# mcychan/nQuant.android

Hardware: AMD Instinct MI355X
Metric: Mpixels/sec, 4096x4096 RGBA -> 256-colour PnnLAB + dither (higher is better)
Workload: dtype f64

## Files before the change

### include/nquant_abi.h

```cpp
#ifndef NQUANT_ABI_H
#define NQUANT_ABI_H
#include <stdint.h>

#ifdef __cplusplus
extern "C" {
#endif

#define NQ_ABI_VERSION 1

typedef struct nq_handle nq_handle;

enum nq_kind { NQ_KIND_RGB = 0,
               NQ_KIND_LAB = 1 };

enum nq_mode {
    NQ_MODE_REFERENCE_SEQUENTIAL = 0,
    NQ_MODE_PARALLEL_TILED = 1,
    NQ_MODE_LOOKUP_ONLY = 2
};

enum nq_status {
    NQ_OK = 0,
    NQ_ERR_INVALID = -1,
    NQ_ERR_HIP = -2,
    NQ_ERR_UNSUPPORTED = -3,
    NQ_ERR_REFERENCE_THROWS = -4,
    NQ_ERR_NO_DEVICE = -5,
    NQ_ERR_TIME_LIMIT = -6
};

typedef struct nq_params {
    int32_t kind;
    int32_t nMaxColors;
    int32_t hasSemiTransparency;
    int32_t transparentPixelIndex;
    int32_t transparentColor;
    int32_t isNano;
    int32_t texicab;
    int32_t quan_rt;
    int32_t maxbins;
    int32_t paletteLength;
    double PR, PG, PB, PA;
    double ratio;
    double weight;
    int64_t distinctColors;
} nq_params;

int nq_create(int kind, int device, nq_handle** out);
void nq_destroy(nq_handle* h);
const char* nq_last_error(const nq_handle* h);
int nq_abi_version(void);
int nq_set_stream(nq_handle* h, void* hip_stream);
int nq_set_tile(nq_handle* h, int tile_w, int tile_h);
int nq_set_band(nq_handle* h, int y0, int image_height);

#define NQ_OPT_CELL_LISTS 1
#define NQ_OPT_FAST_DITHER 2
#define NQ_OPT_DITHER_CHAIN 4
#define NQ_OPT_MERGE_WALL_SECONDS 3
int nq_set_option(nq_handle* h, int option, int value);
int nq_get_dither_path(nq_handle* h, int32_t* out_fast, int32_t* out_failed_tiles);
int nq_get_list_counts(nq_handle* h, uint8_t* closest_counts, uint8_t* nearest_counts);
int nq_selftest_ciede(nq_handle* h, const float* lab_pairs, int64_t n, uint32_t* out9);
#define NQ_FAST_ST_TANH 0
#define NQ_FAST_ST_CLOSEST_ERR 1
#define NQ_FAST_ST_CLOSEST_ERR_PAIRS 2
#define NQ_FAST_ST_NEXTINT 3
#define NQ_FAST_ST_NEXTINT_COUNT 4
#define NQ_FAST_ST_REM 5
#define NQ_FAST_ST_REM_COUNT 6
#define NQ_FAST_ST_YDIFF 7
#define NQ_FAST_ST_YDIFF_RANGE 8
#define NQ_FAST_ST_LAB32 9
#define NQ_FAST_ST_LAB64 10
#define NQ_FAST_ST_NEAR_D32 11
#define NQ_FAST_ST_NEAR_D32_PAIRS 12
#define NQ_FAST_ST_TANH_BITS 13
#define NQ_FAST_ST_NEXTINT_LIST 14
#define NQ_FAST_ST_NEAR_SAFE 15
#define NQ_FAST_ST_MODES 16
int nq_selftest_fast(nq_handle* h, int which, const void* in, int64_t n, uint32_t* out);
int nq_get_params(const nq_handle* h, nq_params* out);
int nq_set_params(nq_handle* h, const nq_params* in);

int nq_gilbert_dither(nq_handle* h, int width, int height, const uint32_t* pixels, const uint32_t* palette, int K,
                      const float* saliencies, double weight, int dither, int64_t rng_seed, int mode,
                      int32_t* out_qpixels, uint16_t* out_index);
int nq_bluenoise_dither(nq_handle* h, int width, int height, const uint32_t* pixels, const uint32_t* palette, int K,
                        int32_t* io_qpixels, float weight, int64_t rng_seed, int mode, uint16_t* out_index);

int nq_convert(nq_handle* h, const uint32_t* argb, int width, int height, int nMaxColors, int dither,
               int64_t rng_seed, int mode,
               uint32_t* out_argb, uint16_t* out_index, uint32_t* out_palette, int32_t* out_K);
int nq_convert_device(nq_handle* h, const uint32_t* d_argb, int width, int height, int nMaxColors, int dither,
                      int64_t rng_seed, int mode,
                      uint32_t* d_out_argb, uint16_t* d_out_index, uint32_t* out_palette, int32_t* out_K);

int nq_convert_batch_device(nq_handle* const* hs, int n, const uint32_t* const* d_argb, const int32_t* widths,
                            const int32_t* heights, int nMaxColors, int dither, const int64_t* rng_seeds, int mode,
                            uint32_t* const* d_out_argb, uint16_t* const* d_out_index,
                            uint32_t* out_palettes, int32_t palette_stride, int32_t* out_K);

int nq_convert_batch(nq_handle* const* hs, int n, const uint32_t* const* argb, const int32_t* widths,
                     const int32_t* heights, int nMaxColors, int dither, const int64_t* rng_seeds, int mode,
                     uint32_t* const* out_argb, uint16_t* const* out_index,
                     uint32_t* out_palettes, int32_t palette_stride, int32_t* out_K);

int nq_pnnquan_frames_device(nq_handle* h, int n, const uint32_t* const* d_argb, const int32_t* widths, const int32_t* heights,
                             int nMaxColors, uint32_t* out_palette, int32_t* out_K);
int nq_convert_frames_device(nq_handle* h, int n, const uint32_t* const* d_argb, const int32_t* widths, const int32_t* heights,
                             int nMaxColors, int dither, const int64_t* rng_seeds, int mode,
                             uint32_t* const* d_out_argb, uint16_t* const* d_out_index,
                             uint32_t* out_palette, int32_t* out_K);
int nq_convert_frames(nq_handle* h, int n, const uint32_t* const* argb, const int32_t* widths, const int32_t* heights,
// ... 239 lines not shown
```

### nquant.android_amd/csrc/nq_abi.cpp

```cpp
#include "../../include/nquant_abi.h"
#include "nq_kernels.h"
#include <hip/hip_runtime.h>
#include <climits>
#include <cmath>
#include <cstdio>
#include <cstdlib>
#include <cstring>
#include <algorithm>
#include <atomic>
#include <map>
#include <string>
#include <utility>
#include <vector>
#include <thread>
#include <exception>

using namespace nq;

static thread_local std::string g_create_error;

namespace {

const float kCoeffs[3][3] = {{0.299f, 0.587f, 0.114f}, {-0.14713f, -0.28886f, 0.436f}, {0.615f, -0.51499f, -0.10001f}};

// ... 100 lines not shown
    out.reserve((size_t) w * h);
    if (w <= 0 || h <= 0) return out;
    if (w >= h) gilbert_rec(out, 0, 0, w, 0, 0, h);
    else gilbert_rec(out, 0, 0, 0, h, w, 0);
    return out;
}

}

struct Scratch {
    DevBuf<unsigned short> keys_a, keys_b;
    DevBuf<int> vals_a, vals_b;
    DevBuf<unsigned char> sort_tmp;
    DevBuf<unsigned> seg;
    DevBuf<double> hist;
    DevBuf<int> init_cand;
    DevBuf<unsigned char> cell_lists;
    DevBuf<float> saliency;
    DevBuf<unsigned> lookup_todo;
    DevBuf<unsigned> dk_a, dk_b, di_a, di_b;
    DevBuf<unsigned char> dtmp;
    DevBuf<unsigned long long> dheads;
    DevBuf<float> cell_box;
    bool cell_box_ready = false;
};

inline size_t path_bytes(int w, int hgt) { const size_t n = (size_t) w * hgt; return (n ? n : 1) * sizeof(uint32_t); }

struct nq_handle {
    int kind = 0, device = 0;
    hipStream_t stream = nullptr;
    std::string err;
    nq_params params;
    int tile_w = 0, tile_h = 0;
    float stage_ms[NQ_N_STAGES] = {0};
    Scratch own;
    Scratch* sc = &own;
    DevBuf<int> d_palette, d_colors, d_tuple;
    DevBuf<uint32_t> d_in, d_out_argb;
    DevBuf<unsigned short> d_out_index;
    DevBuf<short> d_bincache, d_short;
    DevBuf<int> d_seqlog;
    DevBuf<unsigned char> d_seqseen;
    DevBuf<long long> d_scalars;
    DevBuf<int> live3;
    int use_lists = 1;
    int n_cus = 256;
    int merge_wall_s = 0;
    hipStream_t palette_stream = nullptr;
    bool palette_synced = false;
    DevBuf<float> d_user_sal;
    int band_y0 = 0, band_image_h = 0;
    int use_fast_dither = 1;
    int dither_chain_always = 0;
    bool dither_events_fresh = false;
    int last_dither_fast = 0;
    int last_dither_failed_tiles = 0;
    DevBuf<int> d_failed;
    DevBuf<float> scan_f;
    DevBuf<int> scan_i;
    DevBuf<float> scan_box;
    DevBuf<nq::MergeJob> d_jobs;
    DevBuf<int> ring_argb[3];
    DevBuf<unsigned short> ring_index[3];
    hipStream_t copy_stream = nullptr;
    hipStream_t lane_stream = nullptr;
    hipStream_t more_lanes[6] = {nullptr, nullptr, nullptr, nullptr, nullptr, nullptr};
    long long merge_stats[16] = {0};
    std::vector<uint32_t> dev_palette;
    uint32_t* fetched_palette = nullptr; int fetched_len = 0;
    long long merge_readback[37] = {0};
    DevBuf<long long> d_readback;
    long long* h_readback = nullptr; size_t h_readback_words = 0;
    long long* pin = nullptr;
    int merge_variant[2] = {0, 0};
    long long team_stats[16] = {0};
    DevBuf<unsigned long long> team;
    bool light_events = false;
    hipEvent_t bev[4] = {nullptr};
    hipEvent_t lane_gate = nullptr;
    float batch_phase_ms[4] = {0};
    bool ext_distinct_valid = false, ext_distinct_many = false;
    std::vector<int32_t> ext_distinct;
    DevBuf<int> d_ints;
    DevBuf<int> heap;
    std::vector<nq::FrameDesc> h_frames;
    std::vector<nq::FrameChunk> h_items;
    DevBuf<nq::FrameDesc> d_frames;
    DevBuf<nq::FrameChunk> d_items;
    int64_t frames_total = 0;
    bool frames_active = false, reuse_lists = false, lists_built = false;
    nq::ListsView saved_lv;
    unsigned rec_skip = 0;
    std::vector<nq::GifFrame> h_gif;
    DevBuf<nq::GifFrame> d_gif;
    DevBuf<unsigned> gif_words;
    DevBuf<unsigned long long> gif_bits, gif_res;
    DevBuf<unsigned char> gif_blob, gif_file;
    DevBuf<unsigned short> gif_in;
    std::vector<uint8_t> h_gif_blob;
    std::vector<unsigned> h_gif_rgb;
    DevBuf<unsigned> gif_rgb;
    std::vector<int> h_gif_box;
    std::vector<nq::GifDelta> h_gif_delta;
    DevBuf<const unsigned short*> gif_ptrs;
    DevBuf<int> gif_box;
    DevBuf<nq::GifDelta> d_gif_delta;
    DevBuf<unsigned short> gif_body;
    std::vector<nq::GifLocal> h_gif_local;
    DevBuf<nq::GifLocal> d_gif_local;
    std::vector<nq::PngImage> h_png;
    DevBuf<nq::PngImage> d_png;
    DevBuf<unsigned> png_tokens, png_crc;
    DevBuf<unsigned long long> png_adler;
    std::vector<void*> h_hold_ptrs;
    DevBuf<void*> hold_ptrs;
    DevBuf<unsigned long long> hold_held;
    std::vector<const uint32_t*> h_sig_ptrs;
    DevBuf<const uint32_t*> sig_ptrs;
    DevBuf<uint32_t> d_sig;
    std::vector<uint32_t> h_sig;
    std::vector<nq::RefineFrame> h_refine_frames;
    DevBuf<nq::RefineFrame> d_refine_frames;
    std::vector<unsigned long long> h_refine;
    DevBuf<unsigned long long> d_refine;
    std::vector<void*> h_resample_ptrs;
    DevBuf<void*> resample_ptrs;
    std::vector<const void*> h_yuv_ptrs;
    DevBuf<const void*> yuv_ptrs;
    DevBuf<unsigned char> yuv_in;
    std::vector<void*> h_orient_ptrs;
    DevBuf<void*> orient_ptrs;
    DevBuf<uint32_t> orient_tmp;
    std::vector<nq::OrderedFrame> h_ordered_frames;
    DevBuf<nq::OrderedFrame> d_ordered_frames;
    std::vector<unsigned> h_ordered_pal;
    DevBuf<unsigned> d_ordered_pal;
    DevBuf<unsigned long long> d_ordered_stats;
    DevBuf<float> binf;
    DevBuf<double> bind;
    DevBuf<int> bini;
    std::map<std::pair<int, int>, uint32_t*> paths;
    DevBuf<uint32_t> big_path[4];
    int big_w[4] = {0, 0, 0, 0}, big_h[4] = {0, 0, 0, 0};
    hipEvent_t ev[NQ_N_STAGES + 1] = {nullptr};
    bool tables_ready = false;
    ~nq_handle() {
        for (auto& kv : paths) { (void) hipFree(kv.second); g_device_bytes -= (int64_t) path_bytes(kv.first.first, kv.first.second); }
        for (auto& e : ev) if (e) (void) hipEventDestroy(e);
        for (auto& e : bev) if (e) (void) hipEventDestroy(e);
        if (lane_gate) (void) hipEventDestroy(lane_gate);
        if (copy_stream) (void) hipStreamDestroy(copy_stream);
        if (lane_stream) (void) hipStreamDestroy(lane_stream);
        for (auto& ls : more_lanes) if (ls) (void) hipStreamDestroy(ls);
        if (h_readback) (void) hipHostFree(h_readback);
        if (pin) (void) hipHostFree(pin);
    }
};

static inline hipError_t launch_status() {
    const hipError_t a = nq::take_launch_error(), b = hipGetLastError();
    return a != hipSuccess ? a : b;
}

#define NQ_FAIL(h, code, ...) do { char _b[512]; std::snprintf(_b, sizeof _b, __VA_ARGS__); (h)->err = _b; return (code); } while (0)
#define NQ_HIP(h, call) do { hipError_t _e = (call); if (_e != hipSuccess) { \
    NQ_FAIL(h, NQ_ERR_HIP, "%s failed: %s (%s:%d)", #call, hipGetErrorString(_e), __FILE__, __LINE__); } } while (0)

namespace {

int use_device(nq_handle* h) {
    if (!h) return NQ_ERR_INVALID;
    NQ_HIP(h, hipSetDevice(h->device));
    if (!h->tables_ready) {
        double gamma[256];
        for (int ch = 0; ch < 256; ++ch) {
            const double c = ch / 255.0;
            gamma[ch] = c < 0.04045 ? c / 12.92 : std::pow((c + 0.055) / 1.055, 2.4);
        }
        upload_tables(gamma, std::exp(1.5), std::exp(1.75), h->stream);
        upload_tables_fast(gamma, std::exp(1.5), std::exp(1.75), h->stream);
        NQ_HIP(h, launch_status());
        int cus = 0;
        NQ_HIP(h, hipDeviceGetAttribute(&cus, hipDeviceAttributeMultiprocessorCount, h->device));
        if (cus > 0) h->n_cus = cus;
        NQ_HIP(h, h->d_scalars.reserve(64));
        NQ_HIP(h, h->d_ints.reserve(8 + 64));
        NQ_HIP(h, h->d_bincache.reserve(65536));
        if (!h->pin) NQ_HIP(h, hipHostMalloc((void**) &h->pin, 8 * sizeof(long long), hipHostMallocDefault));
        for (auto& e : h->ev) NQ_HIP(h, hipEventCreate(&e));
        for (auto& e : h->bev) NQ_HIP(h, hipEventCreate(&e));
        NQ_HIP(h, hipEventCreateWithFlags(&h->lane_gate, hipEventDisableTiming));
        h->tables_ready = true;
    }
    return NQ_OK;
}

DevParams dev_params(const nq_handle* h, int K) {
    const nq_params& p = h->params;
    DevParams d;
    d.kind = h->kind; d.K = K; d.hasSemi = p.hasSemiTransparency; d.hasAlpha = p.transparentPixelIndex > -1;
    d.transparentColor = p.transparentColor; d.isNano = p.isNano;
    d.binKeyed = h->kind == NQ_KIND_LAB ? (p.isNano != 0) : !(p.weight > .015);
    d.nMaxColors = p.nMaxColors; d.rewriteA0 = p.nMaxColors <= 2 && p.nMaxColors > 0;
    d.pad = 0;
    d.PR = p.PR; d.PG = p.PG; d.PB = p.PB; d.PA = p.PA; d.ratio = p.ratio; d.weight = p.weight;
    return d;
}

int upload_palette(nq_handle* h, const uint32_t* palette, int K) {
    const size_t cap = h->d_palette.n;
    NQ_HIP(h, h->d_palette.reserve((size_t) std::max(K, 2)));
    if (h->d_palette.n != cap) h->dev_palette.clear();
    const bool ordered = h->palette_synced || h->palette_stream == h->stream;
    if (ordered && (int) h->dev_palette.size() == K && std::memcmp(h->dev_palette.data(), palette, (size_t) K * sizeof(uint32_t)) == 0) return NQ_OK;
    h->dev_palette.clear();
    NQ_HIP(h, hipMemcpyAsync(h->d_palette.p, palette, K * sizeof(int), hipMemcpyHostToDevice, h->stream));
    h->dev_palette.assign(palette, palette + K);
    h->palette_stream = h->stream; h->palette_synced = false;
    return NQ_OK;
}
void* packed_lists(nq_handle* h) { return h->sc->cell_lists.p + 2 * (size_t) 65536 * 32 + 2 * 65536; }

int prepare_lists(nq_handle* h, const DevParams& P, nq::ListsView* out, const int* sal_pixels = nullptr, int64_t sal_n = 0, int sal_subst = 0,
                  bool* sal_done = nullptr, int* d_failed = nullptr, bool* failed_cleared = nullptr) {
    if (sal_done) *sal_done = false;
    if (failed_cleared) *failed_cleared = false;
    out->closest = out->closestCount = out->nearest = out->nearestCount = nullptr;
    if (!h->use_lists || P.K > 256 || P.K < 8) return NQ_OK;
    const size_t LB = (size_t) 65536 * 32;
    NQ_HIP(h, h->sc->cell_lists.reserve(2 * LB + 2 * 65536 + 2 * LB));
    unsigned char* base = h->sc->cell_lists.p;
    double wA, wR, wG, wB;
    if (h->kind == NQ_KIND_LAB) {
        double s[3] = {0, 0, 0};
        for (int i = 0; i < 3; ++i) for (int c = 0; c < 3; ++c) s[c] += (double) kCoeffs[i][c] * (double) kCoeffs[i][c];
        wR = P.PR * (1 - P.ratio) + P.ratio * s[0]; wG = P.PG * (1 - P.ratio) + P.ratio * s[1]; wB = P.PB * (1 - P.ratio) + P.ratio * s[2];
        wA = P.hasSemi ? P.PA : 0.0;
    } else {
        double pr = P.PR, pg = P.PG, pb = P.PB, pa = P.PA;
        if (P.K < 3) pr = pg = pb = pa = 1;
        wR = pr; wG = pg; wB = pb; wA = P.hasSemi ? pa : 0.0;
    }
    const bool nearest = h->kind == NQ_KIND_LAB ? (P.K > 32 && !P.hasSemi) : (!P.hasSemi && !P.hasAlpha);
    if (nearest && h->kind == NQ_KIND_LAB && !h->sc->cell_box_ready) {
        NQ_HIP(h, h->sc->cell_box.reserve((size_t) 65536 * 6));
        launch_cell_lab_box(h->sc->cell_box.p, h->stream);
        h->sc->cell_box_ready = true;
    }
    if (sal_pixels) NQ_HIP(h, h->sc->saliency.reserve((size_t) sal_n));
    if (!(h->kind == NQ_KIND_LAB && P.ratio < 0)) { out->closest = base; out->closestCount = base + 2 * LB; }
    if (nearest) { out->nearest = base + LB; out->nearestCount = base + 2 * LB + 65536; }
    const bool pack = h->use_fast_dither && fast_pack_wanted(P, *out);
    bool pack_in_builders = true;
    if (const char* e = std::getenv("NQ_PACK_IN_BUILDERS")) pack_in_builders = std::atoi(e) != 0;
    bool folded = false;
    const bool sal_built = launch_build_lists(P, h->d_palette.p, wA, wR, wG, wB, nearest, h->sc->cell_box.p, base, base + 2 * LB, base + LB,
                                              base + 2 * LB + 65536, h->stream, sal_pixels, sal_n, sal_pixels ? h->sc->saliency.p : nullptr, sal_subst,
                                              pack && pack_in_builders ? packed_lists(h) : nullptr, d_failed, &folded);
    if (sal_done) *sal_done = sal_built;
    if (failed_cleared) *failed_cleared = folded && d_failed;
    if (pack && !(folded && pack_in_builders)) launch_pack_lists(*out, packed_lists(h), h->stream);
    return NQ_OK;
}

int lists_for_call(nq_handle* h, const DevParams& P, nq::ListsView* out, const int* sal_pixels = nullptr, int64_t sal_n = 0, int sal_subst = 0,
                   bool* sal_done = nullptr, int* d_failed = nullptr, bool* failed_cleared = nullptr) {
    if (h->reuse_lists && h->lists_built) {
        if (sal_done) *sal_done = false;
        if (failed_cleared) *failed_cleared = false;
        *out = h->saved_lv;
        return NQ_OK;
    }
    const int rc = prepare_lists(h, P, out, sal_pixels, sal_n, sal_subst, sal_done, d_failed, failed_cleared);
// ... 507 lines not shown
    if (!staged && post && h->kind == NQ_KIND_LAB && !sequential) {
        if (p.distinctColors <= 0) {
            int64_t cnt = 0;
            int rcd = distinct_colors(h, d_argb, n, 0, &cnt, nullptr);
            if (rcd) return rcd;
            p.distinctColors = cnt;
        }
        const double delta = sqr(K) / (double) p.distinctColors;
        blueWeight = delta > 0.023 ? 1.0f : (float) (37.013 * delta + 0.906);
    }
    DevParams P = dev_params(h, K);
    GilbertConsts G = gilbert_consts(K, staged ? ov.weight : p.weight, hasSal, dither != 0);
    G.salSubst = salSubst;

    TileGeom T;
    std::memset(&T, 0, sizeof T);
    T.width = width; T.height = height;
    const bool banded = h->band_image_h > 0;
    if (banded && (sequential || h->band_y0 + height > h->band_image_h))
        NQ_FAIL(h, NQ_ERR_INVALID, "nq_set_band: the band [%d, %d) does not fit the image height %d (or REFERENCE_SEQUENTIAL mode)", h->band_y0, h->band_y0 + height, h->band_image_h);
    const int rule_h = banded ? h->band_image_h : height;
    if (sequential) { T.tile_w = width; T.tile_h = height; }
    else if (h->tile_w > 0 && h->tile_h > 0) { T.tile_w = std::min(h->tile_w, width); T.tile_h = std::min(h->tile_h, rule_h); }
    else {
        int tsz = 4;
        {
            const int cand = 8;
            const int64_t tiles = (int64_t) ((width + cand - 1) / cand) * ((rule_h + cand - 1) / cand);
            if (tiles >= 131072) tsz = cand;
        }
        T.tile_w = std::min(tsz, width); T.tile_h = std::min(tsz, rule_h);
    }
    if (banded) {
        if (h->band_y0 % T.tile_h != 0 || (h->band_y0 + height != h->band_image_h && height % T.tile_h != 0))
            NQ_FAIL(h, NQ_ERR_INVALID, "nq_set_band: band origin %d / rows %d must be multiples of the tile height %d", h->band_y0, height, T.tile_h);
        T.y_origin = h->band_y0;
        T.tile_base = (h->band_y0 / T.tile_h) * ((width + T.tile_w - 1) / T.tile_w);
        T.tile_h = std::min(T.tile_h, height);
    }
    T.tiles_x = (width + T.tile_w - 1) / T.tile_w; T.tiles_y = (height + T.tile_h - 1) / T.tile_h;
    const int rw = width - (T.tiles_x - 1) * T.tile_w, rh = height - (T.tiles_y - 1) * T.tile_h;
    const int sw[4] = {T.tile_w, rw, T.tile_w, rw}, shh[4] = {T.tile_h, T.tile_h, rh, rh};
    for (int s = 0; s < 4; ++s) {
        int rc = get_path(h, sw[s], shh[s], s, &T.path[s]);
        if (rc) return rc;
        T.path_len[s] = sw[s] * shh[s]; T.shape_w[s] = sw[s]; T.shape_h[s] = shh[s];
    }
    if (sequential && !ov.blue_only) NQ_HIP(h, hipMemsetAsync(h->d_bincache.p, 0xFF, 65536 * sizeof(short), h->stream));
    nq::ListsView lv;
    bool sal_done = false;
    const bool want_sal = !staged && hasSal;
    const bool maybe_fast = !ov.blue_only && !sequential && h->use_fast_dither && K > 32 && K <= 256;
    bool failed_cleared = false;
    if (maybe_fast) NQ_HIP(h, h->d_failed.reserve((size_t) T.tiles_x * T.tiles_y + 1));
    { int rcl = lists_for_call(h, P, &lv, want_sal ? (const int*) d_argb : nullptr, n, salSubst ? 1 : 0, &sal_done, maybe_fast ? h->d_failed.p : nullptr,
                               &failed_cleared); if (rcl) return rcl; }
    const float* d_sal = nullptr;
    if (staged) d_sal = hasSal ? ov.d_sal : nullptr;
    else if (hasSal) {
        NQ_HIP(h, h->sc->saliency.reserve((size_t) n));
        if (!sal_done) launch_saliency(P, salSubst ? 1 : 0, (const int*) d_argb, n, h->sc->saliency.p, h->stream);
        d_sal = h->sc->saliency.p;
    }
    rec(h, 5);
    int log_cap = 0;
    if (seq_lab_post) {
        if (3 * n + 16 > 2147483647LL) NQ_FAIL(h, NQ_ERR_INVALID, "image too large for the sequential pixelMap log");
        log_cap = (int) (3 * n + 16);
        NQ_HIP(h, h->d_seqlog.reserve((size_t) log_cap + 4));
        NQ_HIP(h, h->d_seqseen.reserve((size_t) K));
        NQ_HIP(h, hipMemsetAsync(h->d_seqlog.p + log_cap, 0, sizeof(int), h->stream));
        NQ_HIP(h, hipMemsetAsync(h->d_seqseen.p, 0, (size_t) K, h->stream));
    }
    const int* d_tile_list = nullptr;
    h->last_dither_fast = 0;
    if (ov.blue_only) {  }
    else {
    if (!sequential && h->use_fast_dither && gilbert_fast_eligible(P, G, T, lv)) {
        NQ_HIP(h, h->d_failed.reserve((size_t) T.tiles_x * T.tiles_y + 1));
        NQ_HIP(h, launch_gilbert_fast(P, G, T, lv, (const int*) d_argb, d_sal, h->d_palette.p, (long long) seed, d_out_index,
                                      post ? nullptr : (int*) d_out_argb, h->d_failed.p, packed_lists(h), h->stream, failed_cleared,
                                      h->dither_chain_always != 0));
        d_tile_list = h->d_failed.p;
        h->last_dither_fast = 1;
    }
    launch_gilbert(P, G, T, lv, (const int*) d_argb, d_sal, h->d_palette.p, h->d_bincache.p, (long long) seed, sequential ? 1 : 0,
                   h->d_scalars.p, d_out_index, post ? nullptr : (int*) d_out_argb,
                   seq_lab_post ? h->d_seqlog.p : nullptr, seq_lab_post ? h->d_seqlog.p + log_cap : nullptr,
                   seq_lab_post ? h->d_seqseen.p : nullptr, log_cap, d_tile_list, h->stream);
    }
    rec(h, 6);
    if (seq_lab_post) {
        int count = 0;
        NQ_HIP(h, hipMemcpyAsync(&count, h->d_seqlog.p + log_cap, sizeof(int), hipMemcpyDeviceToHost, h->stream));
        NQ_HIP(h, hipStreamSynchronize(h->stream));
        if (count > log_cap) NQ_FAIL(h, NQ_ERR_HIP, "sequential pixelMap log overflow (internal error)");
        std::vector<int32_t> all((size_t) n + count);
        std::vector<unsigned char> seen(K);
        NQ_HIP(h, hipMemcpy(all.data(), d_argb, (size_t) n * sizeof(int), hipMemcpyDeviceToHost));
        if (count) NQ_HIP(h, hipMemcpy(all.data() + n, h->d_seqlog.p, (size_t) count * sizeof(int), hipMemcpyDeviceToHost));
        NQ_HIP(h, hipMemcpy(seen.data(), h->d_seqseen.p, (size_t) K, hipMemcpyDeviceToHost));
        for (int64_t i = 0; i < n; ++i)
            if ((((uint32_t) all[i]) >> 24) <= 0xF) all[i] = p.transparentColor;
        for (int i = 0; i < K; ++i) if (seen[i]) all.push_back((int32_t) palette[i]);
        std::sort(all.begin(), all.end());
        const int64_t distinct = (int64_t) (std::unique(all.begin(), all.end()) - all.begin());
        const double delta = sqr(K) / (double) distinct;
        blueWeight = delta > 0.023 ? 1.0f : (float) (37.013 * delta + 0.906);
    }
    if (post && !sequential && h->use_fast_dither && fast_lookup_eligible(P, lv))
        launch_fast_bluenoise(P, lv, h->d_palette.p, packed_lists(h), (const int*) d_argb, width, height, T.y_origin, blueWeight, (long long) seed,
                              d_out_index, (int*) d_out_argb, h->stream);
    else if (post)
        launch_bluenoise(P, h->d_palette.p, lv, (const int*) d_argb, width, height, T.y_origin, blueWeight, (long long) seed, sequential ? 1 : 0,
                         h->d_bincache.p, h->d_scalars.p, d_out_index, (int*) d_out_argb, h->stream);
    rec(h, 7);
    NQ_HIP(h, launch_status());
    h->dither_events_fresh = true;
    return NQ_OK;
}

void finish_timing(nq_handle* h) {
    for (int i = 0; i < 7; ++i) {
        float ms = 0;
        if (h->light_events && i != 5) { h->stage_ms[i] = -1.0f; continue; }
        if (hipEventElapsedTime(&ms, h->ev[i], h->ev[i + 1]) != hipSuccess) ms = 0;
        h->stage_ms[i] = ms;
    }
    float tot = 0;
    if (hipEventElapsedTime(&tot, h->ev[0], h->ev[h->light_events ? 6 : 7]) != hipSuccess) tot = 0;
    h->stage_ms[7] = tot;
    h->dither_events_fresh = false;
}

void finish_batch_timing(nq_handle* h0) {
    for (int i = 0; i < 3; ++i) {
        float ms = 0;
        if (hipEventElapsedTime(&ms, h0->bev[i], h0->bev[i + 1]) != hipSuccess) ms = 0;
        h0->batch_phase_ms[i] = ms;
    }
    float tot = 0;
    if (hipEventElapsedTime(&tot, h0->bev[0], h0->bev[3]) != hipSuccess) tot = 0;
// ... 108 lines not shown
    if (!host) return refine_device(h, n, argb, widths, heights, total, io_palette, K, iterations, out_sse, out_counts, out_passes);
    return host_form(h, [&]() -> int {
        std::vector<const uint32_t*> d_src(n);
        size_t room = 0;
        for (int i = 0; i < n; ++i) room += ((size_t) widths[i] * heights[i] + 3) & ~(size_t) 3;
        NQ_HIP(h, h->d_in.reserve(room));
        size_t at = 0;
        for (int i = 0; i < n; ++i) {
            const size_t px = (size_t) widths[i] * heights[i];
            d_src[i] = h->d_in.p + at;
            NQ_HIP(h, hipMemcpyAsync(h->d_in.p + at, argb[i], px * sizeof(uint32_t), hipMemcpyHostToDevice, h->stream));
            at += (px + 3) & ~(size_t) 3;
        }
        return refine_device(h, n, d_src.data(), widths, heights, total, io_palette, K, iterations, out_sse, out_counts, out_passes);
    });
}

int refine_check_convert(nq_handle* h, int refine, int nMaxColors) {
    if (refine < 0 || refine > 64) NQ_FAIL(h, NQ_ERR_INVALID, "refine = %d: must be 0..64", refine);
    if (refine > 0 && nMaxColors > 256) NQ_FAIL(h, NQ_ERR_INVALID, "refine needs nMaxColors <= 256");
    return NQ_OK;
}

int batch_check(nq_handle* const* hs, int n, const uint32_t* const* argb, const int32_t* widths, const int32_t* heights, int nMaxColors,
                const int64_t* rng_seeds, uint32_t* const* out_argb, const uint32_t* out_palettes, int32_t palette_stride, const int32_t* out_K,
                bool host) {
    nq_handle* h0 = hs[0];
    if (!argb || !widths || !heights || !rng_seeds || !out_argb || !out_palettes || !out_K) NQ_FAIL(h0, NQ_ERR_INVALID, "bad argument");
    if (palette_stride < std::max(nMaxColors, 2)) NQ_FAIL(h0, NQ_ERR_INVALID, "palette_stride < max(nMaxColors, 2)");
    for (int i = 0; i < n; ++i) {
        if (host && (!hs[i] || !argb[i] || !out_argb[i] || widths[i] <= 0 || heights[i] <= 0)) NQ_FAIL(h0, NQ_ERR_INVALID, "bad argument for image %d", i);
        if (!hs[i]) NQ_FAIL(h0, NQ_ERR_INVALID, "null handle in batch");
        if (hs[i]->device != h0->device) NQ_FAIL(h0, NQ_ERR_INVALID, "handles of a batch must share one device");
        for (int j = 0; j < i; ++j) if (hs[j] == hs[i]) NQ_FAIL(h0, NQ_ERR_INVALID, "a handle appears twice in the batch");
    }
    return NQ_OK;
}

int batch_fail(nq_handle* h0, nq_handle* h, int rc) { if (h != h0) h0->err = h->err; return rc; }

int batch_use_device(nq_handle* const* hs, int n) {
    for (int i = 0; i < n; ++i) {
        int rc = use_device(hs[i]);
        if (rc) return batch_fail(hs[0], hs[i], rc);
        if (i) NQ_HIP(hs[0], hipStreamSynchronize(hs[i]->stream));
    }
    return NQ_OK;
}

struct BatchGuard {
    nq_handle* const* hs; int n;
    std::vector<hipStream_t> streams;
    std::vector<hipEvent_t> events;
    BatchGuard(nq_handle* const* hh, int nn) : hs(hh), n(nn) { for (int i = 0; i < n; ++i) streams.push_back(hs[i]->stream); }
    ~BatchGuard() {
        for (int i = 0; i < n; ++i) { hs[i]->stream = streams[i]; hs[i]->sc = &hs[i]->own; hs[i]->light_events = false; }
        for (hipEvent_t e : events) (void) hipEventDestroy(e);
    }
};

int color_lookup(nq_handle* h, const uint32_t* palette, int K, const uint32_t* colors, int64_t M, int16_t* out_index, int32_t* out_closest4) {
    int rc = use_device(h);
    if (rc) return rc;
    if (!palette || K < 1 || K > 8192 || !colors || M < 0 || !(out_index || out_closest4)) NQ_FAIL(h, NQ_ERR_INVALID, "bad argument");
    if (M == 0) return NQ_OK;
    const size_t m = (size_t) M, m4 = 4 * m;
    return host_form(h, [&]() -> int {
        int* d_colors = nullptr;
        int16_t* d_index = nullptr;
        int32_t* d_tuple = nullptr;
        rc = upload_palette(h, palette, K);
        if (!rc) rc = out_index ? stage_room(h, h->d_short, 1, &m, &d_index) : stage_room(h, h->d_tuple, 1, &m4, &d_tuple);
        if (!rc) rc = stage_in(h, h->d_colors, 1, &m, &colors, &d_colors);
        DevParams P = dev_params(h, K);
        nq::ListsView lv;
        if (!rc) rc = prepare_lists(h, P, &lv);
        if (rc) return rc;
        const bool fast = h->use_fast_dither && fast_lookup_eligible(P, lv);
        if (d_index && fast) launch_fast_nearest_index(P, lv, h->d_palette.p, packed_lists(h), d_colors, M, d_index, h->stream);
        else if (d_index) launch_nearest_index(P, h->d_palette.p, lv, d_colors, M, d_index, h->stream);
        else if (fast) launch_fast_closest_tuple(P, lv, h->d_palette.p, packed_lists(h), d_colors, M, d_tuple, h->stream);
        else launch_closest_tuple(P, h->d_palette.p, lv, d_colors, M, d_tuple, h->stream);
        NQ_HIP(h, launch_status());
        rc = out_index ? stage_out(h, h->d_short, 1, &m, &out_index) : stage_out(h, h->d_tuple, 1, &m4, &out_closest4);
        if (rc) return rc;
        NQ_HIP(h, hipStreamSynchronize(h->stream));
        return NQ_OK;
    });
}

}

extern "C" {

int nq_abi_version(void) { return NQ_ABI_VERSION; }

int nq_create(int kind, int device, nq_handle** out) {
    if (!out) { g_create_error = "out is NULL"; return NQ_ERR_INVALID; }
    *out = nullptr;
    if (kind != NQ_KIND_RGB && kind != NQ_KIND_LAB) { g_create_error = "unknown kind"; return NQ_ERR_INVALID; }
    int count = 0;
    hipError_t e = hipGetDeviceCount(&count);
    if (e != hipSuccess || count <= 0) {
        g_create_error = "no HIP device available (libnquant_hip has no CPU fallback)";
        return NQ_ERR_NO_DEVICE;
    }
    if (device < 0 || device >= count) { g_create_error = "device ordinal out of range"; return NQ_ERR_INVALID; }
    nq_handle* h = new nq_handle();
    h->kind = kind; h->device = device;
    std::memset(&h->params, 0, sizeof h->params);
    h->params.kind = kind; h->params.transparentPixelIndex = -1; h->params.transparentColor = (int32_t) 0x00FFFFFFu;
    h->params.PR = 0.299; h->params.PG = 0.587; h->params.PB = 0.114; h->params.PA = .3333; h->params.ratio = .5; h->params.weight = 1;
    int rc = use_device(h);
    if (rc) { g_create_error = h->err; delete h; return rc; }
    *out = h;
    return NQ_OK;
}

void nq_destroy(nq_handle* h) {
    if (!h) return;
    (void) hipSetDevice(h->device);
    (void) hipStreamSynchronize(h->stream);
    delete h;
}

const char* nq_last_error(const nq_handle* h) { return h ? h->err.c_str() : g_create_error.c_str(); }

int nq_set_stream(nq_handle* h, void* hip_stream) {
    if (!h) return NQ_ERR_INVALID;
    h->stream = (hipStream_t) hip_stream;
    return NQ_OK;
}
int nq_set_tile(nq_handle* h, int tile_w, int tile_h) {
    if (!h) return NQ_ERR_INVALID;
    if (tile_w <= 0 || tile_h <= 0) { tile_w = 0; tile_h = 0; }
    h->tile_w = tile_w; h->tile_h = tile_h;
    return NQ_OK;
}
int nq_set_band(nq_handle* h, int y0, int image_height) {
    if (!h) return NQ_ERR_INVALID;
    if (y0 < 0 || image_height < 0 || (image_height == 0 && y0 != 0) || (image_height > 0 && y0 >= image_height))
        NQ_FAIL(h, NQ_ERR_INVALID, "nq_set_band: bad origin %d / image height %d", y0, image_height);
    h->band_y0 = y0; h->band_image_h = image_height;
    return NQ_OK;
}
int nq_get_list_counts(nq_handle* h, uint8_t* closest_counts, uint8_t* nearest_counts) {
    if (!h || !closest_counts || !nearest_counts) return NQ_ERR_INVALID;
    if (!h->sc->cell_lists.p) NQ_FAIL(h, NQ_ERR_INVALID, "no lists built yet");
    const size_t LB = (size_t) 65536 * 32;
    NQ_HIP(h, hipMemcpy(closest_counts, h->sc->cell_lists.p + 2 * LB, 65536, hipMemcpyDeviceToHost));
    NQ_HIP(h, hipMemcpy(nearest_counts, h->sc->cell_lists.p + 2 * LB + 65536, 65536, hipMemcpyDeviceToHost));
    return NQ_OK;
}
int nq_set_option(nq_handle* h, int option, int value) {
    if (!h) return NQ_ERR_INVALID;
    if (option == NQ_OPT_CELL_LISTS) { h->use_lists = value != 0; return NQ_OK; }
    if (option == NQ_OPT_FAST_DITHER) { h->use_fast_dither = value != 0; return NQ_OK; }
    if (option == NQ_OPT_DITHER_CHAIN) { h->dither_chain_always = value != 0; return NQ_OK; }
    if (option == NQ_OPT_MERGE_WALL_SECONDS) { h->merge_wall_s = value > 0 ? value : 0; return NQ_OK; }
    NQ_FAIL(h, NQ_ERR_INVALID, "unknown option %d", option);
}
int nq_selftest_ciede(nq_handle* h, const float* lab_pairs, int64_t n, uint32_t* out9) {
    int rc = use_device(h);
    if (rc) return rc;
    if (!lab_pairs || n <= 0 || !out9) NQ_FAIL(h, NQ_ERR_INVALID, "bad argument");
    float* d_in = nullptr; unsigned* d_out = nullptr;
    NQ_HIP(h, hipMalloc((void**) &d_in, (size_t) n * 6 * sizeof(float)));
    hipError_t e = hipMalloc((void**) &d_out, (size_t) n * 9 * sizeof(unsigned));
    if (e == hipSuccess) e = hipMemcpyAsync(d_in, lab_pairs, (size_t) n * 6 * sizeof(float), hipMemcpyHostToDevice, h->stream);
    if (e == hipSuccess) { launch_ciede_selftest(d_in, n, d_out, h->stream); e = hipGetLastError(); }
    if (e == hipSuccess) e = hipMemcpyAsync(out9, d_out, (size_t) n * 9 * sizeof(unsigned), hipMemcpyDeviceToHost, h->stream);
    if (e == hipSuccess) e = hipStreamSynchronize(h->stream);
    (void) hipFree(d_in); if (d_out) (void) hipFree(d_out);
    if (e != hipSuccess) NQ_FAIL(h, NQ_ERR_HIP, "nq_selftest_ciede: %s", hipGetErrorString(e));
    return NQ_OK;
}
int nq_selftest_fast(nq_handle* h, int which, const void* in, int64_t n, uint32_t* out) {
    int rc = use_device(h);
    if (rc) return rc;
    if (which < 0 || which >= NQ_FAST_ST_MODES || !in || n <= 0 || !out) NQ_FAIL(h, NQ_ERR_INVALID, "nq_selftest_fast: bad argument");
    static const struct { int rec_bytes, out_words; int64_t domain; } k_mode[] = {
        {0, 2, (int64_t) 1 << 32}, {0, 3, 1 << 24}, {8, 3, 0}, {0, 1, (int64_t) 1 << 31}, {0, 0, (int64_t) 1 << 31}, {8, 1, 0}, {0, 0, 1 << 30},
        {24, 3, 0}, {0, 3, 1 << 24}, {0, 3, 1 << 24}, {0, 3, 1 << 24}, {0, 1, 1 << 24}, {8, 1, 0}, {4, 2, 0}, {4, 1, 0}, {8, 1, 0}};
    static_assert(sizeof k_mode / sizeof k_mode[0] == NQ_FAST_ST_MODES && NQ_FAST_ST_MODES == NQ_FAST_ST_NEAR_SAFE + 1, "one row per NQ_FAST_ST_* mode, in their order");
    const auto& m = k_mode[which];
    const bool counting = m.out_words == 0;
    if (!counting && n > ((int64_t) 1 << 26)) NQ_FAIL(h, NQ_ERR_INVALID, "nq_selftest_fast: more than 2^26 elements in one call");
    int64_t first = 0, a0 = 0, a1 = 0;
    const void* up = in;
    size_t up_bytes = (size_t) n * (size_t) m.rec_bytes;
    if (m.rec_bytes == 0) {
        const int64_t* hdr = (const int64_t*) in;
        first = hdr[0]; a0 = hdr[2]; a1 = hdr[3];
        if (hdr[1] != n || first < 0 || first > m.domain || n > m.domain - first) NQ_FAIL(h, NQ_ERR_INVALID, "nq_selftest_fast: range outside the domain");
        up = nullptr;
        if (which == NQ_FAST_ST_CLOSEST_ERR && (a0 < 0 || a0 > 7)) NQ_FAIL(h, NQ_ERR_INVALID, "nq_selftest_fast: sign mask");
        if (which == NQ_FAST_ST_YDIFF_RANGE) {
            if (a1 < 0 || (a1 >> 1) > 32) NQ_FAIL(h, NQ_ERR_INVALID, "nq_selftest_fast: more than 32 thresholds");
            up = hdr + 4; up_bytes = (size_t) (a1 >> 1) * sizeof(double);
        }
    }
    const bool wants_palette = which == NQ_FAST_ST_NEAR_D32 || which == NQ_FAST_ST_NEAR_D32_PAIRS || which == NQ_FAST_ST_NEAR_SAFE;
    const int K = (int) h->dev_palette.size();
    if (wants_palette && (K < 1 || K > 256 || !h->d_palette.p)) NQ_FAIL(h, NQ_ERR_INVALID, "nq_selftest_fast: no palette of at most 256 entries on the device (run a lookup first)");
    if (which == NQ_FAST_ST_NEAR_D32 && (a0 < 0 || a0 >= K)) NQ_FAIL(h, NQ_ERR_INVALID, "nq_selftest_fast: palette index");
    const DevParams P = dev_params(h, wants_palette ? K : 0);
    const size_t out_bytes = counting ? 16 : (size_t) n * (size_t) m.out_words * sizeof(uint32_t);
    const uint64_t count_init[2] = {0, ~(uint64_t) 0};
    void* d_in = nullptr; unsigned* d_out = nullptr;
    hipError_t e = hipMalloc((void**) &d_out, out_bytes);
    if (e == hipSuccess && up_bytes) e = hipMalloc(&d_in, up_bytes);
    if (e == hipSuccess && up_bytes) e = hipMemcpyAsync(d_in, up, up_bytes, hipMemcpyHostToDevice, h->stream);
    if (e == hipSuccess && counting) e = hipMemcpyAsync(d_out, count_init, 16, hipMemcpyHostToDevice, h->stream);
    if (e == hipSuccess) { launch_fast_selftest(P, wants_palette ? h->d_palette.p : nullptr, which, d_in, first, n, a0, a1, d_out, h->stream); e = hipGetLastError(); }
    if (e == hipSuccess) e = hipMemcpyAsync(out, d_out, out_bytes, hipMemcpyDeviceToHost, h->stream);
    if (e == hipSuccess) e = hipStreamSynchronize(h->stream);
    if (d_in) (void) hipFree(d_in);
    if (d_out) (void) hipFree(d_out);
    if (e != hipSuccess) NQ_FAIL(h, NQ_ERR_HIP, "nq_selftest_fast: %s", hipGetErrorString(e));
    return NQ_OK;
}
int nq_get_dither_path(nq_handle* h, int32_t* out_fast, int32_t* out_failed_tiles) {
    if (!h) return NQ_ERR_INVALID;
    if (out_fast) *out_fast = h->last_dither_fast;
    if (out_failed_tiles) {
        *out_failed_tiles = 0;
        if (h->last_dither_fast && h->d_failed.p) {
            NQ_HIP(h, hipStreamSynchronize(h->stream));
            int cnt = 0;
            NQ_HIP(h, hipMemcpy(&cnt, h->d_failed.p, sizeof(int), hipMemcpyDeviceToHost));
            *out_failed_tiles = cnt;
        }
    }
    return NQ_OK;
}
int nq_get_params(const nq_handle* h, nq_params* out) {
    if (!h || !out) return NQ_ERR_INVALID;
    *out = h->params;
    return NQ_OK;
}
int nq_set_params(nq_handle* h, const nq_params* in) {
    if (!h || !in) return NQ_ERR_INVALID;
    h->params = *in; h->params.kind = h->kind;
    return NQ_OK;
}
int nq_get_merge_stats(const nq_handle* h, int64_t* out8) {
    if (!h || !out8) return NQ_ERR_INVALID;
    std::memcpy(out8, h->merge_stats, 16 * sizeof(long long));
    return NQ_OK;
}
int nq_get_team_stats(const nq_handle* h, int64_t* out16) {
    if (!h || !out16) return NQ_ERR_INVALID;
    std::memcpy(out16, h->team_stats, sizeof h->team_stats);
    return NQ_OK;
}
int nq_get_device_bytes(int64_t* out) {
    if (!out) return NQ_ERR_INVALID;
    *out = g_device_bytes.load();
    return NQ_OK;
}
int nq_get_merge_variant(const nq_handle* h, int32_t* out_threads, int32_t* out_helpers) {
    if (!h || !out_threads || !out_helpers) return NQ_ERR_INVALID;
    *out_threads = h->merge_variant[0]; *out_helpers = h->merge_variant[1];
    return NQ_OK;
}
int nq_get_batch_phase_ms(const nq_handle* h0, float* out4) {
    if (!h0 || !out4) return NQ_ERR_INVALID;
    std::memcpy(out4, h0->batch_phase_ms, sizeof h0->batch_phase_ms);
    return NQ_OK;
}
int nq_get_stage_ms(const nq_handle* h, float* out8) {
    if (!h || !out8) return NQ_ERR_INVALID;
    std::memcpy(out8, h->stage_ms, sizeof h->stage_ms);
    if (h->dither_events_fresh) {
        float ms = 0;
        if (hipEventElapsedTime(&ms, h->ev[5], h->ev[6]) == hipSuccess) out8[5] = ms;
        if (hipEventElapsedTime(&ms, h->ev[6], h->ev[7]) == hipSuccess) out8[6] = ms;
    }
    return NQ_OK;
}

int nq_pnnquan_device(nq_handle* h, const uint32_t* d_argb, int width, int height, int nMaxColors,
                      uint32_t* out_palette, int32_t* out_K) {
    int rc = use_device(h);
    if (rc) return rc;
    return pnnquan_device(h, d_argb, width, height, nMaxColors, out_palette, out_K);
// ... 140 lines not shown
        int64_t cnt = 0;
        rc = distinct_colors(h, nullptr, total, 0, &cnt, nullptr);
        if (rc) return rc;
        p.distinctColors = cnt;
    }
    h->frames_active = false;
    h->reuse_lists = true;
    for (int i = 0; i < n; ++i) {
        if (n > 1) h->rec_skip = i == 0 ? (1u << 6 | 1u << 7) : (1u << 5 | 1u << 6 | 1u << 7);
        rc = dither_device(h, d_argb[i], widths[i], heights[i], out_palette, K, dither, rng_seeds[i], mode, d_out_argb[i],
                           d_out_index ? d_out_index[i] : nullptr);
        if (rc) { h->err = "frame " + std::to_string(i) + ": " + h->err; return rc; }
    }
    h->rec_skip = 0;
    if (n > 1) { rec(h, 6); rec(h, 7); }
    NQ_HIP(h, hipStreamSynchronize(h->stream));
    finish_timing(h);
    return NQ_OK;
}

int nq_convert_frames_device(nq_handle* h, int n, const uint32_t* const* d_argb, const int32_t* widths, const int32_t* heights,
                             int nMaxColors, int dither, const int64_t* rng_seeds, int mode,
                             uint32_t* const* d_out_argb, uint16_t* const* d_out_index, uint32_t* out_palette, int32_t* out_K) {
    return nq_convert_frames_refined_device(h, n, d_argb, widths, heights, nMaxColors, 0, dither, rng_seeds, mode, d_out_argb, d_out_index,
                                            out_palette, out_K);
}

int nq_convert_frames_refined(nq_handle* h, int n, const uint32_t* const* argb, const int32_t* widths, const int32_t* heights,
                              int nMaxColors, int refine, int dither, const int64_t* rng_seeds, int mode,
                              uint32_t* const* out_argb, uint16_t* const* out_index, uint32_t* out_palette, int32_t* out_K) {
    if (!h) return NQ_ERR_INVALID;
    int rc = frames_check(h, n, argb, widths, heights, nMaxColors, true, nullptr);
    if (rc) return rc;
    rc = refine_check_convert(h, refine, nMaxColors);
    if (rc) return rc;
    if (!out_argb || !rng_seeds || !out_palette || !out_K) NQ_FAIL(h, NQ_ERR_INVALID, "bad argument");
    for (int i = 0; i < n; ++i) if (!out_argb[i]) NQ_FAIL(h, NQ_ERR_INVALID, "frame %d: null output pointer", i);
    rc = check_mode(h, mode);
    if (rc) return rc;
    rc = use_device(h);
    if (rc) return rc;
    std::vector<size_t> px(n);
    for (int i = 0; i < n; ++i) px[i] = (size_t) widths[i] * heights[i];
    return host_images(h, n, px.data(), argb, out_argb, out_index, [&](auto in, auto out, auto index) {
        return nq_convert_frames_refined_device(h, n, in, widths, heights, nMaxColors, refine, dither, rng_seeds, mode, out, index, out_palette,
                                                out_K);
    });
}

int nq_convert_frames(nq_handle* h, int n, const uint32_t* const* argb, const int32_t* widths, const int32_t* heights,
                      int nMaxColors, int dither, const int64_t* rng_seeds, int mode,
                      uint32_t* const* out_argb, uint16_t* const* out_index, uint32_t* out_palette, int32_t* out_K) {
    return nq_convert_frames_refined(h, n, argb, widths, heights, nMaxColors, 0, dither, rng_seeds, mode, out_argb, out_index, out_palette, out_K);
}

int nq_convert_batch_device(nq_handle* const* hs, int n, const uint32_t* const* d_argb, const int32_t* widths, const int32_t* heights,
                            int nMaxColors, int dither, const int64_t* rng_seeds, int mode,
                            uint32_t* const* d_out_argb, uint16_t* const* d_out_index,
                            uint32_t* out_palettes, int32_t palette_stride, int32_t* out_K) {
    if (!hs || n <= 0 || !hs[0]) return NQ_ERR_INVALID;
    nq_handle* h0 = hs[0];
    int rc = batch_check(hs, n, d_argb, widths, heights, nMaxColors, rng_seeds, d_out_argb, out_palettes, palette_stride, out_K, false);
    if (rc) return rc;
    BatchGuard guard(hs, n);
    for (int i = 0; i < n; ++i) hs[i]->light_events = i >= 16;
    rc = batch_use_device(hs, n);
    if (rc) return rc;
    if (n > 1 && !h0->lane_stream) NQ_HIP(h0, hipStreamCreateWithFlags(&h0->lane_stream, hipStreamNonBlocking));
    int L = std::min(n, 4);
    if (const char* f = std::getenv("NQ_BATCH_LANES")) { const int t = std::atoi(f); if (t >= 1 && t <= 8) L = std::min(t, n); }
    hipStream_t lane_s[8] = {h0->stream, n > 1 ? h0->lane_stream : h0->stream, nullptr, nullptr, nullptr, nullptr, nullptr, nullptr};
    Scratch* lane_sc[8] = {&h0->own, n > 1 ? &hs[1]->own : &h0->own, nullptr, nullptr, nullptr, nullptr, nullptr, nullptr};
    for (int k = 2; k < L; ++k) {
        if (!h0->more_lanes[k - 2]) NQ_HIP(h0, hipStreamCreateWithFlags(&h0->more_lanes[k - 2], hipStreamNonBlocking));
        lane_s[k] = h0->more_lanes[k - 2]; lane_sc[k] = &hs[k]->own;
    }
    for (int i = 0; i < n; ++i) { hs[i]->stream = lane_s[i % L]; hs[i]->sc = lane_sc[i % L]; }
    std::vector<PaletteJob> jobs(n);
    std::vector<const PaletteJob*> jp(n);
    (void) hipEventRecord(h0->bev[0], lane_s[0]);
    for (int k = 1; k < L; ++k)
        if (lane_s[k] != lane_s[0]) {
            if (k == 1) NQ_HIP(h0, hipEventRecord(h0->lane_gate, lane_s[0]));
            NQ_HIP(h0, hipStreamWaitEvent(lane_s[k], h0->lane_gate, 0));
        }
    {
        std::vector<int> lane_rc(L, NQ_OK), lane_bad(L, -1);
        auto lane_work = [&](int k) {
            int at = k;
            try {
                if (hipSetDevice(h0->device) != hipSuccess) { lane_rc[k] = NQ_ERR_HIP; lane_bad[k] = k; hs[k]->err = "hipSetDevice failed in a batch lane"; return; }
                for (int i = k; i < n; i += L) {
                    at = i;
                    const int rc = pnnquan_prepare(hs[i], d_argb[i], widths[i], heights[i], nMaxColors, out_palettes + (size_t) i * palette_stride,
                                                   out_K + i, &jobs[i]);
                    if (rc) { lane_rc[k] = rc; lane_bad[k] = i; return; }
                    jp[i] = &jobs[i];
                }
                const hipError_t e = launch_status();
                if (e != hipSuccess) {
                    lane_rc[k] = NQ_ERR_HIP; lane_bad[k] = at;
                    hs[at]->err = std::string("launch_status() failed in a batch lane: ") + hipGetErrorString(e);
                }
            } catch (const std::exception& e) {
                lane_rc[k] = NQ_ERR_HIP; lane_bad[k] = at;
                try { hs[at]->err = std::string("exception in a batch lane: ") + e.what(); } catch (...) {}
            } catch (...) { lane_rc[k] = NQ_ERR_HIP; lane_bad[k] = at; }
        };
        std::vector<std::thread> workers;
        std::vector<int> inline_lanes;
        for (int k = 1; k < L; ++k) {
            try { workers.emplace_back(lane_work, k); } catch (const std::exception&) { inline_lanes.push_back(k); }
        }
        lane_work(0);
        for (int k : inline_lanes) lane_work(k);
        for (auto& t : workers) t.join();
        if (std::any_of(lane_rc.begin(), lane_rc.end(), [](int r) { return r != NQ_OK; }))
            for (int k = 0; k < L; ++k) (void) hipStreamSynchronize(lane_s[k]);
        for (int k = 0; k < L; ++k)
            if (lane_rc[k]) return batch_fail(h0, hs[lane_bad[k] >= 0 && lane_bad[k] < n ? lane_bad[k] : 0], lane_rc[k]);
    }
    for (int k = 1; k < L; ++k) NQ_HIP(h0, hipStreamSynchronize(lane_s[k]));
    (void) hipEventRecord(h0->bev[1], lane_s[0]);
    std::vector<int> order;
    rc = merge_launch(h0, jp.data(), n, &order);
    if (rc) return rc;
    (void) hipEventRecord(h0->bev[2], lane_s[0]);
    for (int i = 0; i < n; ++i) { hs[i]->stream = lane_s[0]; hs[i]->sc = lane_sc[0]; }
    for (int i = 0; i < n; ++i) if (jobs[i].merge) rec(hs[i], 4);
    const size_t n_jobs = order.size();
    size_t slot_words = 0;
    if (n_jobs) {
        int max_plen = 0;
        for (int i : order) max_plen = std::max(max_plen, jobs[i].plen);
        slot_words = 37 + ((size_t) max_plen + 1) / 2;
        NQ_HIP(h0, h0->d_readback.reserve(n_jobs * slot_words));
        if (h0->h_readback_words < n_jobs * slot_words) {
            if (h0->h_readback) { (void) hipHostFree(h0->h_readback); h0->h_readback = nullptr; h0->h_readback_words = 0; }
            NQ_HIP(h0, hipHostMalloc((void**) &h0->h_readback, n_jobs * slot_words * sizeof(long long), hipHostMallocDefault));
            h0->h_readback_words = n_jobs * slot_words;
        }
        nq::launch_merge_readback(h0->d_jobs.p, (int) n_jobs, h0->d_readback.p, (long long) slot_words, lane_s[0]);
        NQ_HIP(h0, hipMemcpyAsync(h0->h_readback, h0->d_readback.p, n_jobs * slot_words * sizeof(long long), hipMemcpyDeviceToHost, lane_s[0]));
    }
    NQ_HIP(h0, hipStreamSynchronize(lane_s[0]));
    NQ_HIP(h0, launch_status());
    for (size_t j = 0; j < n_jobs; ++j) {
        const int i = order[j];
        const long long* slot = h0->h_readback + j * slot_words;
        uint32_t* pal = out_palettes + (size_t) i * palette_stride;
        std::memcpy(hs[i]->merge_readback, slot, sizeof hs[i]->merge_readback);
        std::memcpy(pal, slot + 37, (size_t) jobs[i].plen * sizeof(uint32_t));
        hs[i]->fetched_palette = pal; hs[i]->fetched_len = jobs[i].plen;
    }
    for (int i = 0; i < n; ++i)
        if (jobs[i].merge) {
            rc = palette_check(hs[i], jobs[i], out_K + i);
            if (rc) return batch_fail(h0, hs[i], rc);
        }
    for (int i = 0; i < n; ++i) {
        uint32_t* pal = out_palettes + (size_t) i * palette_stride;
        rc = dither_device(hs[i], d_argb[i], widths[i], heights[i], pal, out_K[i], dither, rng_seeds[i], mode, d_out_argb[i],
                           d_out_index ? d_out_index[i] : nullptr);
        if (rc) return batch_fail(h0, hs[i], rc);
    }
    (void) hipEventRecord(h0->bev[3], lane_s[0]);
    NQ_HIP(h0, hipStreamSynchronize(lane_s[0]));
    for (int i = 0; i < n; ++i) finish_timing(hs[i]);
    finish_batch_timing(h0);
    return NQ_OK;
}

int nq_convert_batch(nq_handle* const* hs, int n, const uint32_t* const* argb, const int32_t* widths, const int32_t* heights,
                     int nMaxColors, int dither, const int64_t* rng_seeds, int mode,
                     uint32_t* const* out_argb, uint16_t* const* out_index,
                     uint32_t* out_palettes, int32_t palette_stride, int32_t* out_K) {
    if (!hs || n <= 0 || !hs[0]) return NQ_ERR_INVALID;
    nq_handle* h0 = hs[0];
    int rc = batch_check(hs, n, argb, widths, heights, nMaxColors, rng_seeds, out_argb, out_palettes, palette_stride, out_K, true);
    if (rc) return rc;
    BatchGuard guard(hs, n);
    rc = batch_use_device(hs, n);
    if (rc) return rc;
    size_t max_px = 0;
    for (int i = 0; i < n; ++i) {
        max_px = std::max(max_px, (size_t) widths[i] * heights[i]);
        NQ_HIP(h0, hs[i]->d_in.reserve((size_t) widths[i] * heights[i]));
        hs[i]->stream = h0->stream; hs[i]->sc = &h0->own;
    }
    constexpr int RING = 3;
    for (int r = 0; r < RING; ++r) { NQ_HIP(h0, h0->ring_argb[r].reserve(max_px)); NQ_HIP(h0, h0->ring_index[r].reserve(max_px)); }
    if (!h0->copy_stream) NQ_HIP(h0, hipStreamCreateWithFlags(&h0->copy_stream, hipStreamNonBlocking));
    hipStream_t cs = h0->copy_stream;
    auto new_event = [&](hipEvent_t* e) -> hipError_t {
        hipError_t rc = hipEventCreateWithFlags(e, hipEventDisableTiming);
        if (rc == hipSuccess) guard.events.push_back(*e);
        return rc;
    };
    std::vector<hipEvent_t> ev_up(n), ev_done(n), ev_dl(n);
    for (int i = 0; i < n; ++i) { NQ_HIP(h0, new_event(&ev_up[i])); NQ_HIP(h0, new_event(&ev_done[i])); NQ_HIP(h0, new_event(&ev_dl[i])); }
    int uploaded = 0;
    auto upload_until = [&](int last) -> int {
        for (; uploaded <= last && uploaded < n; ++uploaded) {
            const int i = uploaded;
            NQ_HIP(h0, hipMemcpyAsync(hs[i]->d_in.p, argb[i], (size_t) widths[i] * heights[i] * sizeof(int), hipMemcpyHostToDevice, cs));
            NQ_HIP(h0, hipEventRecord(ev_up[i], cs));
        }
        return NQ_OK;
    };
    std::vector<PaletteJob> jobs(n);
    std::vector<const PaletteJob*> jp(n);
    (void) hipEventRecord(h0->bev[0], h0->stream);
    for (int i = 0; i < n; ++i) {
        rc = upload_until(i + 2);
        if (rc) return rc;
        NQ_HIP(h0, hipStreamWaitEvent(h0->stream, ev_up[i], 0));
        rc = pnnquan_prepare(hs[i], hs[i]->d_in.p, widths[i], heights[i], nMaxColors,
                             out_palettes + (size_t) i * palette_stride, out_K + i, &jobs[i]);
        if (rc) return batch_fail(h0, hs[i], rc);
        jp[i] = &jobs[i];
    }
    (void) hipEventRecord(h0->bev[1], h0->stream);
    rc = merge_launch(h0, jp.data(), n);
    if (rc) return rc;
    (void) hipEventRecord(h0->bev[2], h0->stream);
    for (int i = 0; i < n; ++i) if (jobs[i].merge) rec(hs[i], 4);
    for (int i = 0; i < n; ++i) {
        uint32_t* pal = out_palettes + (size_t) i * palette_stride;
        if (jobs[i].merge) {
            rc = palette_finish(hs[i], jobs[i], pal, out_K + i);
            if (rc) return batch_fail(h0, hs[i], rc);
        }
        const int r = i % RING;
        if (i >= RING) NQ_HIP(h0, hipStreamWaitEvent(h0->stream, ev_dl[i - RING], 0));
        rc = dither_device(hs[i], hs[i]->d_in.p, widths[i], heights[i], pal, out_K[i], dither, rng_seeds[i], mode,
                           (uint32_t*) h0->ring_argb[r].p, h0->ring_index[r].p);
        if (rc) return batch_fail(h0, hs[i], rc);
        NQ_HIP(h0, hipEventRecord(ev_done[i], h0->stream));
        NQ_HIP(h0, hipStreamWaitEvent(cs, ev_done[i], 0));
        const size_t px = (size_t) widths[i] * heights[i];
        NQ_HIP(h0, hipMemcpyAsync(out_argb[i], h0->ring_argb[r].p, px * sizeof(int), hipMemcpyDeviceToHost, cs));
        if (out_index && out_index[i])
            NQ_HIP(h0, hipMemcpyAsync(out_index[i], h0->ring_index[r].p, px * sizeof(uint16_t), hipMemcpyDeviceToHost, cs));
        NQ_HIP(h0, hipEventRecord(ev_dl[i], cs));
    }
    (void) hipEventRecord(h0->bev[3], h0->stream);
    NQ_HIP(h0, hipStreamSynchronize(h0->stream));
    NQ_HIP(h0, hipStreamSynchronize(cs));
    for (int i = 0; i < n; ++i) finish_timing(hs[i]);
    finish_batch_timing(h0);
    return NQ_OK;
}

int nq_convert(nq_handle* h, const uint32_t* argb, int width, int height, int nMaxColors, int dither,
               int64_t rng_seed, int mode, uint32_t* out_argb, uint16_t* out_index, uint32_t* out_palette, int32_t* out_K) {
    int rc = use_device(h);
    if (rc) return rc;
    if (!argb || !out_argb || width <= 0 || height <= 0) NQ_FAIL(h, NQ_ERR_INVALID, "bad argument");
    const size_t px = (size_t) width * height;
    return host_images(h, 1, &px, &argb, &out_argb, &out_index, [&](auto in, auto out, auto index) {
        return nq_convert_device(h, in[0], width, height, nMaxColors, dither, rng_seed, mode, out[0], index[0], out_palette, out_K);
    });
}

int nq_nearest_index(nq_handle* h, const uint32_t* palette, int K, const uint32_t* colors, int64_t M, int16_t* out_index) {
    return color_lookup(h, palette, K, colors, M, out_index, nullptr);
}

int nq_closest_tuple(nq_handle* h, const uint32_t* palette, int K, const uint32_t* colors, int64_t M, int32_t* out_closest4) {
    return color_lookup(h, palette, K, colors, M, nullptr, out_closest4);
}

int nq_band_scan_device(nq_handle* h, const uint32_t* d_argb, int64_t n_pixels, int64_t index_offset, int nMaxColors, int64_t* d_scan3) {
    int rc = use_device(h);
    if (rc) return rc;
    if (!d_argb || n_pixels <= 0 || !d_scan3) NQ_FAIL(h, NQ_ERR_INVALID, "bad argument");
    (void) nMaxColors;
    launch_prescan((const int*) d_argb, n_pixels, index_offset, (long long*) d_scan3, h->stream);
    NQ_HIP(h, launch_status());
    return NQ_OK;
}

int nq_set_scan(nq_handle* h, int nMaxColors, int64_t transparent_index, uint32_t transparent_color, int64_t semi_count) {
    if (!h) return NQ_ERR_INVALID;
    apply_scan(h, nMaxColors, transparent_index, transparent_color, semi_count);
    h->ext_distinct_valid = false; h->ext_distinct_many = false; h->ext_distinct.clear();
    return NQ_OK;
}

int nq_band_distinct_device(nq_handle* h, const uint32_t* d_argb, int64_t n_pixels, int cap, int64_t* out_count, uint32_t* out_colors) {
    int rc = use_device(h);
    if (rc) return rc;
    if (!d_argb || n_pixels <= 0 || cap < 1 || !out_count || !out_colors) NQ_FAIL(h, NQ_ERR_INVALID, "bad argument");
    std::vector<int32_t> cols;
    rc = distinct_colors(h, d_argb, n_pixels, cap, out_count, &cols);
    if (rc) return rc;
    if (*out_count <= cap) std::memcpy(out_colors, cols.data(), cols.size() * sizeof(int32_t));
    return NQ_OK;
// ... 2757 lines not shown
```

### nquant.android_amd/csrc/nq_dither.inc

```

namespace nq {

__device__ __forceinline__ int load_pixel(const DevParams& P, const int* __restrict__ pixels, long long i) {
    int c = pixels[i];
    if (P.rewriteA0 && c_alpha(c) == 0) c = P.transparentColor;
    return c;
}

__global__ void __launch_bounds__(256) nearest_index_kernel(DevParams P, const int* __restrict__ g_palette, CellLists lists,
                                                            const int* __restrict__ colors, long long M, short* __restrict__ out) {
    extern __shared__ __align__(16) unsigned char smem[];
    PalView pal = stage_palette(P, g_palette, smem);
    for (long long i = (long long) blockIdx.x * blockDim.x + threadIdx.x; i < M; i += (long long) gridDim.x * blockDim.x)
        out[i] = (short) nearest_any(P, pal, colors[i], &lists);
}

__global__ void __launch_bounds__(256) closest_tuple_kernel(DevParams P, const int* __restrict__ g_palette, CellLists lists,
                                                            const int* __restrict__ colors, long long M, int* __restrict__ out4) {
    extern __shared__ __align__(16) unsigned char smem[];
    PalView pal = stage_palette(P, g_palette, smem);
    for (long long i = (long long) blockIdx.x * blockDim.x + threadIdx.x; i < M; i += (long long) gridDim.x * blockDim.x) {
        int c = colors[i];
        int closest[4];
        if (c_alpha(c) <= 0xF) closest[0] = closest[1] = closest[2] = closest[3] = -1;
// ... 80 lines not shown
        }
        q.set(k, x, xy);
    }
}

struct ChainCtx {
    const DevParams* P;
    const GilbertConsts* G;
    LookupCtx lk;
    const int* pixels;
    const float* saliency;
    int width;
    int gofs;
    int yorg;
    const float* weights;
    int nweights;
};

__device__ __forceinline__ float saliency_lds(int c, const double* __restrict__ gam) {
    const double Y = 100 * (gam[c_red(c)] * 0.2126 + gam[c_green(c)] * 0.7152 + gam[c_blue(c)] * 0.0722);
    const float L = (float) fmax(0.0, 116 * pivot_xyz_fast(Y / 100.0) - 16);
    return .1f + (1 - .1f) * L / 100.0f * (float) c_alpha(c) / 255.0f;
}
__device__ __forceinline__ void saliency_body(const DevParams& P, int salSubst, const int* __restrict__ pixels, long long N,
                                              float* __restrict__ out, long long vec4, int block, int nblocks, double* gam ) {
    gam[threadIdx.x] = g_tab.gamma[threadIdx.x];
    __syncthreads();
    auto fix = [&](int pixel) -> int {
        if (P.rewriteA0 && c_alpha(pixel) == 0) pixel = P.transparentColor;
        if (salSubst && c_alpha(pixel) <= 0xF) pixel = P.transparentColor;
        return pixel;
    };
    const long long stride = (long long) nblocks * blockDim.x, t0 = (long long) block * blockDim.x + threadIdx.x;
    for (long long g = t0; g < vec4; g += stride) {
        const int4 p = reinterpret_cast<const int4*>(pixels)[g];
        float4 r;
        r.x = saliency_lds(fix(p.x), gam); r.y = saliency_lds(fix(p.y), gam); r.z = saliency_lds(fix(p.z), gam); r.w = saliency_lds(fix(p.w), gam);
        reinterpret_cast<float4*>(out)[g] = r;
    }
    for (long long i = 4 * vec4 + t0; i < N; i += stride) out[i] = saliency_lds(fix(pixels[i]), gam);
}
__global__ void __launch_bounds__(256) saliency_kernel(DevParams P, int salSubst, const int* __restrict__ pixels, long long N,
                                                       float* __restrict__ out, long long vec4) {
    __shared__ double gam[256];
    saliency_body(P, salSubst, pixels, N, out, vec4, (int) blockIdx.x, (int) gridDim.x, gam);
}

__global__ void __launch_bounds__(256) build_lab_lists_kernel(DevParams P, const int* __restrict__ g_palette, double wA, double wR, double wG,
                                                              double wB, int kstart, const float* __restrict__ box,
                                                              unsigned char* __restrict__ closest, unsigned char* __restrict__ closestCount,
                                                              unsigned char* __restrict__ nearest, unsigned char* __restrict__ nearestCount, SalJob sal,
                                                              void* packed, int* failed) {
    extern __shared__ __align__(16) unsigned char smem[];
    if (failed && blockIdx.x == 0 && threadIdx.x == 0) failed[0] = 0;
    if (blockIdx.x < 256) closest_lists_body(P, g_palette, wA, wR, wG, wB, closest, closestCount, (int) blockIdx.x, packed);
    else if (blockIdx.x < 512) nearest_lists_body(P, g_palette, kstart, box, nearest, nearestCount, (int) blockIdx.x - 256, smem, packed);
    else saliency_body(P, sal.salSubst, sal.pixels, sal.N, sal.out, sal.vec4, (int) blockIdx.x - 512, sal.blocks, reinterpret_cast<double*>(smem));
}


__device__ __forceinline__ int ditherPixelColor(ChainCtx& cx, int x, int y, int c2, float beta, int pixel, float sal, int qcurIdx) {
    const DevParams& P = *cx.P;
    const GilbertConsts& G = *cx.G;
    const int K = P.K;
    const int bidx = x + y * cx.width;
    const double* __restrict__ gam = cx.lk.pal.gamma;
    const signed char* __restrict__ blue = cx.lk.pal.blue;
    const int qcur = cx.lk.pal.argb[qcurIdx];
    const int r_pix = c_red(c2), g_pix = c_green(c2), b_pix = c_blue(c2), a_pix = c_alpha(c2);
    const double weight = G.weightAbs;
    const float strength = 1 / 3.0f;
    const int acceptedDiff = max(2, K - G.margin);
    const double yPixel = color2Y_t(pixel, gam);
    if (K <= 4 && sal > .2f && sal < .25f)
        c2 = blue_diffuse_t(pixel, qcur, beta * 2 / sal, strength, x, y, blue);
    else if (K <= 4 || Y_Diff_y(yPixel, color2Y_t(c2, gam)) < (2 * acceptedDiff)) {
        if (K > 64) {
            float kappa = sal < .6f ? beta * .15f / sal : beta * .4f / sal;
            c2 = blue_diffuse_t(pixel, qcur, kappa, strength, x, y, blue);
        }
        else if (K > 16 && weight < .005)
            c2 = blue_diffuse_t(pixel, qcur, beta * normalDistribution(sal, .5f) + beta, strength, x, y, blue);
        else
            c2 = blue_diffuse_t(pixel, qcur, beta * .5f / sal, strength, x, y, blue);
    }
    double gamma = (K <= 32 && weight < .01 && weight > .007) ? 1 - beta : beta;
    if (K > 4 && Y_Diff_y(yPixel, color2Y_t(c2, gam)) > (gamma * acceptedDiff)) {
        if (G.margin > 6 || gamma > beta) {
            float kappa = sal < .4f ? beta * .4f * sal : beta * .4f / sal;
            int c1 = c_argb(a_pix, r_pix, g_pix, b_pix);
            if (K > 32 && sal < .9)
                kappa = beta * normalDistribution(sal, 2.0f);
            else {
                if (weight >= .0015 && sal < .6) c1 = pixel;
                if (weight >= .005 && sal < .6)
                    kappa = beta * normalDistribution(sal, weight < .0008 ? 2.5f : 1.75f);
                else if (K >= 32 || Y_Diff_y(color2Y_t(c1, gam), color2Y_t(c2, gam)) > (gamma * NQ_PI * acceptedDiff)) {
                    double ub = 1 - K / 320.0;
                    if (sal > .15 && sal < ub)
                        kappa = beta * (!G.sortedByYDiff && weight < .0025 ? .55f : .5f) / sal;
                    else
                        kappa = beta * normalDistribution(sal, weight < .0025 ? 1.82f : 2.0f);
                }
            }
            c2 = blue_diffuse_t(c1, qcur, kappa, strength, x, y, blue);
        }
        else if (K <= 32 && weight >= .004)
// ... 263 lines not shown
```

### nquant.android_amd/csrc/nq_dither_fast.hip

```cpp
#include "nq_device.h"
#include "nq_kernels.h"
#include "../../include/nquant_abi.h"
#include <cstring>
#include <cmath>
#include <cstdlib>


namespace nq {

struct FastArgs {
    float qa, qb, qc;
    float limiterDiv;
    int strideBytes;
    int failedCap;
    int vecOut;
    int* failed;
    const uint4* packed;
    const uint4* cont;
    int debug;
    int chainAlways;
};
#ifdef NQ_FAST_MARKS
#define NQ_MARK(name) asm volatile("; MARK " name)
#else
#define NQ_MARK(name)
#endif
#ifdef NQ_FAST_KNOCKOUT
#define NQ_KO(bit) (F.debug & (bit))
#else
#define NQ_KO(bit) false
#endif

#ifdef NQ_FAST_COUNT
enum { FC_NEAREST = 0, FC_NEAREST_EXACT, FC_NEAREST_EXACT_LANES, FC_NEAREST_EXACT_N2_SUM, FC_NEAREST_EXACT_N2_MAX, FC_NEAREST_TAIL, FC_CLOSEST,
       FC_CLOSEST_TAIL, FC_CLOSEST_EXACT, FC_YDIFF, FC_YDIFF_F64, FC_TANH, FC_TANH_LIBRARY, FC_CHAIN_LIGHT, FC_CHAIN_REWALK,
       FC_SLOTS = 16 };
__device__ unsigned long long g_fast_count[FC_SLOTS];
__device__ __forceinline__ void fast_count_add(int slot, bool cond, unsigned long long v, bool use_max) {
    const unsigned long long active = __ballot(1), m = __ballot(cond);
    if (!m) return;
    unsigned long long r = 0ULL;
    for (unsigned long long mm = m; mm; mm &= mm - 1) {
        const unsigned long long o = (unsigned) __builtin_amdgcn_readlane((int) v, __ffsll((long long) mm) - 1);
        r = use_max ? (o > r ? o : r) : r + o;
    }
    if ((int) (threadIdx.x & 63) == __ffsll((long long) active) - 1) atomicAdd(&g_fast_count[slot], r);
}
#define NQ_COUNT(slot, cond) do { if (__ballot(cond) && (int) (threadIdx.x & 63) == __ffsll((long long) __ballot(1)) - 1) atomicAdd(&g_fast_count[slot], 1ULL); } while (0)
#define NQ_COUNT_SUM(slot, cond, v) fast_count_add(slot, cond, (unsigned long long) (v), false)
#define NQ_COUNT_MAX(slot, cond, v) fast_count_add(slot, cond, (unsigned long long) (v), true)
#else
#define NQ_COUNT(slot, cond)
#define NQ_COUNT_SUM(slot, cond, v)
#define NQ_COUNT_MAX(slot, cond, v)
#endif

#define NQ_FAST_W(t) __uint_as_float(k_fast_w25[t])
static constexpr unsigned k_fast_w25[25] = {
    0x3a24fc7du, 0x3a5271d1u, 0x3a8636c6u, 0x3aab3193u, 0x3ada5cbdu, 0x3b0b437au, 0x3b31a273u, 0x3b6293edu, 0x3b9080cfu, 0x3bb8515cu,
    0x3beb1a3eu, 0x3c15f09cu, 0x3c3f40a4u, 0x3c73f2a9u, 0x3c9b94c7u, 0x3cc672b7u, 0x3cfd2047u, 0x3d216f47u, 0x3d4dea18u, 0x3d835325u,
    0x3da78228u, 0x3dd5a962u, 0x3e084405u, 0x3e2dcf89u, 0x3e5db34bu};
bool fast_weights_match(const float* w25) {
    for (int i = 0; i < 25; ++i) { unsigned u; std::memcpy(&u, &w25[i], 4); if (u != k_fast_w25[i]) return false; }
    return true;
}

__global__ void __launch_bounds__(256) pack_lists_kernel(CellLists L, uint4* __restrict__ out, uint4* __restrict__ cont) {
    const int cell = blockIdx.x * blockDim.x + threadIdx.x;
    if (cell >= 65536) return;
    __align__(16) unsigned char rec[32];
    __align__(16) unsigned char more[32];
    for (int half = 0; half < 2; ++half) {
        const unsigned char* src = (half ? L.nearest : L.closest) + (size_t) cell * NQ_LIST_CAP;
// ... 358 lines not shown
                }
            }
            if (peak > 0.f) kappa = beta * normal_distribution_cold(sal, peak);
            c2 = blue_diffuse_t(c1, qcur, kappa, strength, x, y, S.blue);
        }
        else c2 = c_in;
    }
    if (sal > .95) {
        const float kappa = beta * fmaxf(.05f, .75f - K / 128.0f) * sal;
        c2 = blue_diffuse_t(pixel, qcur, kappa, strength, x, y, S.blue);
    }
    return c2;
}

template <int U>
__device__ __forceinline__ void fast_accumulate(const float (&q)[NQ_FQ][4], float (&e)[4], float& maxErr) {
#pragma unroll
    for (int t = 0; t < 25; ++t) {
        const float w = NQ_FAST_W(t);
#pragma unroll
        for (int j = 0; j < 4; ++j) e[j] = e[j] + q[U + t][j] * w;
        maxErr = fmaxf(fmaxf(maxErr, e[0]), e[1]);
        maxErr = fmaxf(fmaxf(maxErr, e[2]), e[3]);
    }
    asm volatile("; window offset %0" :: "n"(U));
}

#define NQ_MARK_L(name) do { if (LIGHT) NQ_MARK("light_" name); else NQ_MARK(name); } while (0)
template <bool LIGHT>
__device__ __forceinline__ int fast_lab_index(const FastLds& S, const FastLookup& X, const FastArgs& F, int K, int c, long long& rng, bool& failed) {
    int qidx = 0;
    if (c_alpha(c) <= 0xF) failed = true;
    else {
        const int cell = NQ_KO(1) ? 0 : cell_of(c);
        const uint4 la = X.packed[2 * cell], na = X.packed[2 * cell + 1];
        const int ncl = (int) (la.w >> 24), nnr = (int) (na.w >> 24);
        if (ncl == 255 || nnr == 255) failed = true;
        const int n1 = (ncl == 255 || NQ_KO(16)) ? 0 : ncl, n2 = nnr == 255 ? 0 : nnr;
        NQ_MARK_L("lists_fetched");
        const FastClosest t = fast_closest_tuple(S, X, c, la, n1, cell);
        NQ_MARK_L("closest_done");
        const int idx = fast_closest_pick(t, rng);
        const int ci = idx ? t.c1 : t.c0, ei = idx ? t.e1 : t.e0;
        qidx = ci;
        NQ_MARK_L("picked");
        if ((ei >= K || ci == 0 || c_alpha(S.argb[ci]) < c_alpha(c)) && !NQ_KO(2)) {
            qidx = fast_nearest(S, X, c, na, n2, cell);
        }
        NQ_MARK_L("nearest_done");
    }
    return qidx;
}

template <int MINWAVES, int KIND = 1>
__global__ void __launch_bounds__(256, MINWAVES) gilbert_fast_kernel(DevParams P, GilbertConsts G, TileGeom T, CellLists lists, FastArgs F,
                                                                      const int* __restrict__ pixels, const float* __restrict__ saliency,
                                                                      const int* __restrict__ g_palette, long long seed,
                                                                      unsigned short* __restrict__ out_index, int* __restrict__ out_argb) {
    extern __shared__ __align__(16) unsigned char smem[];
    const int tilepx = T.tile_w * T.tile_h;
    FastLds S;
    {
        unsigned char* p = smem;
        S.argb = (const int*) p; p += 256 * 4;
        S.lab = (const float4*) p; p += 256 * 16;
        S.gamma = (const double*) p; p += 256 * 8;
        S.gamma32 = (const float*) p; p += 256 * 4;
        S.blue = (const signed char*) p; p += 4096;
        S.path = (const unsigned*) p; p += (size_t) 4 * tilepx * 4;
        S.tileinfo = (int4*) p; p += 256 * 16;
        S.stage = p;
    }
    const int K = P.K;
    const int tid = threadIdx.x;
    {
        int* a = (int*) S.argb; float4* l = (float4*) S.lab; double* g = (double*) S.gamma; float* g32 = (float*) S.gamma32;
        int c2 = tid < K ? g_palette[tid] : 0;
        a[tid] = c2;
        if (KIND == 1) {
            const Lab l2 = RGB2LAB(c2);
            l[tid] = make_float4(l2.L, l2.A, l2.B, 0.f);
        }
        g[tid] = g_tab.gamma[tid];
        g32[tid] = (float) g_tab.gamma[tid];
        for (int i = tid; i < 1024; i += 256) ((int*) S.blue)[i] = ((const int*) g_tab.blue)[i];
        unsigned* pp = (unsigned*) S.path;
        for (int s = 0; s < 4; ++s)
            for (int i = tid; i < tilepx; i += 256) pp[s * tilepx + i] = i < T.path_len[s] ? T.path[s][i] : 0u;
    }

    const int ntiles = T.tiles_x * T.tiles_y;
    const int tile = blockIdx.x * 256 + tid;
    const bool live = tile < ntiles;
    const int ty = live ? tile / T.tiles_x : 0, tx = live ? tile - ty * T.tiles_x : 0;
    const int shape = (tx == T.tiles_x - 1 ? 1 : 0) | (ty == T.tiles_y - 1 ? 2 : 0);
    const int steps = live ? T.path_len[shape] : 0;
    const int x0 = tx * T.tile_w, y0 = ty * T.tile_h;
    S.tileinfo[tid] = make_int4(x0, y0, live ? T.shape_w[shape] : 0, live ? T.shape_h[shape] : 0);
    __syncthreads();

    const unsigned* __restrict__ path = S.path + shape * tilepx;
    unsigned char* stage = S.stage + (size_t) tid * F.strideBytes;
    const int width = T.width;
    long long rng = jr_seed((long long) mix64((unsigned long long) seed + (unsigned long long) (T.tile_base + tile)));
    const int gofs = T.y_origin * width;
    const bool branchA = KIND == 1 && G.hasSaliencies && G.dither;
    const bool hasSal = KIND == 1 && G.hasSaliencies != 0;
    const double rpa = P.PA, rpr = P.PR, rpg = P.PG, rpb = P.PB;
    FastLookup X;
    X.packed = F.packed; X.cont = F.cont; X.qa = F.qa; X.qb = F.qb; X.qc = F.qc;
    X.ratio = P.ratio; X.wr = P.PR * (1 - P.ratio); X.wg = P.PG * (1 - P.ratio); X.wb = P.PB * (1 - P.ratio);
    X.kfirst = P.hasAlpha ? 1 : 0;
    const float ditherMaxF = (float) G.ditherMax, ditherMax1 = (float) (G.ditherMax - 1);
    const bool illusionAll = S.blue[0] > G.thresold;
    bool failed = false;

    unsigned d_next = 0;
    int bidx_next = 0, pixel_next = 0;
    float sal_next = 0.f;
    const int maxsteps = T.path_len[0];

    bool rewalk = true;
    if (KIND == 1 && branchA && 2 * max(2, K - G.margin) > 100 && !F.chainAlways) {
        rewalk = false;
        if (steps > 0) {
            d_next = path[0];
            bidx_next = (x0 + (int) (d_next & 0xFFFFu)) + (y0 + (int) (d_next >> 16)) * width;
            pixel_next = pixels[bidx_next];
            sal_next = saliency[bidx_next];
        }
        for (int s = 0; s < maxsteps; ++s) {
            bool need = false;
            int c = 0, pos = 0;
            if (s < steps) {
                const int pixel = pixel_next;
                const float sal = sal_next;
                const int dxx = (int) (d_next & 0xFFFFu), dyy = (int) (d_next >> 16);
                const int xx = x0 + dxx, yy = y0 + dyy + T.y_origin;
                pos = dyy * T.tile_w + dxx;
                if (s + 1 < steps) {
                    d_next = path[s + 1];
                    bidx_next = (x0 + (int) (d_next & 0xFFFFu)) + (y0 + (int) (d_next >> 16)) * width;
                    pixel_next = pixels[bidx_next];
                    sal_next = saliency[bidx_next];
                }
                NQ_MARK("light_begin");
                need = K >= 256 && sal > .99f;
                if (!need) c = fast_dither_color<true>(S, G, K, xx, yy, 0, pixel, sal, need);
                NQ_MARK("light_color");
            }
            if (__ballot(need)) { rewalk = true; break; }
            if (s < steps) {
                const int qidx = fast_lab_index<true>(S, X, F, K, c, rng, failed);
                stage[pos] = (unsigned char) qidx;
                NQ_MARK("light_end");
            }
        }
        NQ_COUNT(FC_CHAIN_LIGHT, live && !rewalk);
        NQ_COUNT(FC_CHAIN_REWALK, live && rewalk);
        if (rewalk) rng = jr_seed((long long) mix64((unsigned long long) seed + (unsigned long long) (T.tile_base + tile)));
    }

    float q[NQ_FQ][4];
#pragma unroll
    for (int t = 0; t < NQ_FQ; ++t) { q[t][0] = q[t][1] = q[t][2] = q[t][3] = 0.f; }

    if (rewalk && steps > 0) {
        d_next = path[0];
        bidx_next = (x0 + (int) (d_next & 0xFFFFu)) + (y0 + (int) (d_next >> 16)) * width;
        pixel_next = pixels[bidx_next];
        if (hasSal) sal_next = saliency[bidx_next];
    }
    if (rewalk)
    for (int s = 0; s < maxsteps; ++s) {
        const int u = s % 5;
        if (s < steps) {
            const int bidx = bidx_next;
            const int pixel = pixel_next;
            const float sal = sal_next;
            const int dxx = (int) (d_next & 0xFFFFu), dyy = (int) (d_next >> 16);
            const int xx = x0 + dxx, yy = y0 + dyy + T.y_origin, pos = dyy * T.tile_w + dxx;
            if (s + 1 < steps) {
                d_next = path[s + 1];
                bidx_next = (x0 + (int) (d_next & 0xFFFFu)) + (y0 + (int) (d_next >> 16)) * width;
                pixel_next = pixels[bidx_next];
                if (hasSal) sal_next = saliency[bidx_next];
            }

            NQ_MARK("step_begin");
            float e[4] = {(float) c_red(pixel), (float) c_green(pixel), (float) c_blue(pixel), (float) c_alpha(pixel)};
            float maxErr = 24.0f;
            if (!NQ_KO(32))
            switch (u) {
                case 0: fast_accumulate<0>(q, e, maxErr); break;
                case 1: fast_accumulate<1>(q, e, maxErr); break;
                case 2: fast_accumulate<2>(q, e, maxErr); break;
                case 3: fast_accumulate<3>(q, e, maxErr); break;
                default: fast_accumulate<4>(q, e, maxErr); break;
            }
            const int r_pix = (int) fminf(255.0f, fmaxf(e[0], 0.0f));
            const int g_pix = (int) fminf(255.0f, fmaxf(e[1], 0.0f));
            const int b_pix = (int) fminf(255.0f, fmaxf(e[2], 0.0f));
            const int a_pix = (int) fminf(255.0f, fmaxf(e[3], 0.0f));
            const int c2 = c_argb(a_pix, r_pix, g_pix, b_pix);
            NQ_MARK("accumulated");

            int c = c2;
            bool unused = false;
            if (branchA && !(K >= 256 && sal > .99f) && !NQ_KO(8)) c = fast_dither_color<false>(S, G, K, xx, yy, c2, pixel, sal, unused);
            NQ_MARK("dither_color");

            int qidx = 0;
            if (KIND == 0) {
                if (c_alpha(c) != 255) failed = true;
                else {
                    const int cell = cell_of(c);
                    const uint4 na = X.packed[2 * cell + 1];
                    const int nnr = (int) (na.w >> 24);
                    if (nnr == 255) failed = true;
                    else qidx = fast_nearest_rgb(S, rpa, rpr, rpg, rpb, c, na, nnr, X.cont + 65536 + cell);
                }
            }
            else qidx = fast_lab_index<false>(S, X, F, K, c, rng, failed);

            const int cq = S.argb[qidx];
            e[0] = (float) (r_pix - c_red(cq));
            e[1] = (float) (g_pix - c_green(cq));
            e[2] = (float) (b_pix - c_blue(cq));
            e[3] = (float) (a_pix - c_alpha(cq));
            const bool diffuse = S.blue[(bidx + gofs) & 4095] > G.thresold;
            NQ_MARK("error_formed");
            {
                float ea = e[0], eb = e[1], ec = e[2];
#pragma unroll 1
                for (int j = 0; j < 3; ++j) {
                    if (fabsf(ea) >= ditherMaxF && !NQ_KO(4)) {
                        if (diffuse) ea = tanh_to_float(ea / maxErr * 20) * ditherMax1;
                        else if (illusionAll) ea = (ea / maxErr) * ditherMax1;
                        else ea /= F.limiterDiv;
                    }
                    const float tmp = ea; ea = eb; eb = ec; ec = tmp;
                }
                e[0] = ea; e[1] = eb; e[2] = ec;
            }
            NQ_MARK("limited");
            switch (u) {
                case 0: q[25][0] = e[0]; q[25][1] = e[1]; q[25][2] = e[2]; q[25][3] = e[3]; asm volatile("; push 0"); break;
                case 1: q[26][0] = e[0]; q[26][1] = e[1]; q[26][2] = e[2]; q[26][3] = e[3]; asm volatile("; push 1"); break;
                case 2: q[27][0] = e[0]; q[27][1] = e[1]; q[27][2] = e[2]; q[27][3] = e[3]; asm volatile("; push 2"); break;
                case 3: q[28][0] = e[0]; q[28][1] = e[1]; q[28][2] = e[2]; q[28][3] = e[3]; asm volatile("; push 3"); break;
                default:
#pragma unroll
                    for (int t = 0; t < 20; ++t) {
#pragma unroll
                        for (int j = 0; j < 4; ++j) q[t][j] = q[t + 5][j];
                    }
#pragma unroll
                    for (int t = 20; t < 24; ++t) {
#pragma unroll
                        for (int j = 0; j < 4; ++j) q[t][j] = q[t + 5][j];
                    }
                    q[24][0] = e[0]; q[24][1] = e[1]; q[24][2] = e[2]; q[24][3] = e[3];
                    break;
            }
            stage[pos] = (unsigned char) qidx;
            NQ_MARK("step_end");
        }
    }

    if (failed && live) {
        const int slot = atomicAdd(F.failed, 1);
        if (slot < F.failedCap) F.failed[1 + slot] = tile;
    }
    __syncthreads();

    {
        const int wave = tid >> 6, lane = tid & 63;
        const unsigned char* wstage = S.stage + (size_t) (wave * 64) * F.strideBytes;
        const int4* winfo = S.tileinfo + wave * 64;
        const int tw = T.tile_w, th = T.tile_h;
        if (F.vecOut) {
            const int gpr = tw >> 2;
            for (int r = 0; r < th; ++r)
                for (int it = 0; it < gpr; ++it) {
                    const int g = it * 64 + lane;
                    const int t = g / gpr, cgrp = (g - t * gpr) * 4;
                    const int4 ti = winfo[t];
                    if (r < ti.w && cgrp < ti.z) {
                        const unsigned kk = *reinterpret_cast<const unsigned*>(wstage + (size_t) t * F.strideBytes + r * tw + cgrp);
                        const long long bidx = (long long) (ti.y + r) * width + ti.x + cgrp;
                        const unsigned k0 = kk & 0xFF, k1 = (kk >> 8) & 0xFF, k2 = (kk >> 16) & 0xFF, k3 = kk >> 24;
                        uint2 iv; iv.x = k0 | (k1 << 16); iv.y = k2 | (k3 << 16);
                        *reinterpret_cast<uint2*>(out_index + bidx) = iv;
                        if (out_argb) *reinterpret_cast<int4*>(out_argb + bidx) = make_int4(S.argb[k0], S.argb[k1], S.argb[k2], S.argb[k3]);
                    }
                }
        } else {
            for (int r = 0; r < th; ++r)
                for (int it = 0; it < tw; ++it) {
                    const int g = it * 64 + lane;
                    const int t = g / tw, cc = g - t * tw;
                    const int4 ti = winfo[t];
                    if (r < ti.w && cc < ti.z) {
                        const int k = wstage[(size_t) t * F.strideBytes + r * tw + cc];
                        const long long bidx = (long long) (ti.y + r) * width + ti.x + cc;
                        out_index[bidx] = (unsigned short) k;
                        if (out_argb) out_argb[bidx] = S.argb[k];
                    }
                }
        }
    }
}


struct FastLookupLds { FastLds S; PalView pal; };
__device__ __forceinline__ FastLookupLds fast_stage_lookup(const DevParams& P, const int* __restrict__ g_palette) {
    __shared__ __align__(16) int s_argb[256];
    __shared__ __align__(16) float4 s_lab[256];
    __shared__ __align__(16) double s_gamma[256];
    __shared__ float s_gamma32[256];
    __shared__ float s_L[256], s_A[256], s_B[256];
    const int tid = threadIdx.x;
    const int c2 = tid < P.K ? g_palette[tid] : 0;
    s_argb[tid] = c2;
    const Lab l2 = RGB2LAB(c2);
    s_lab[tid] = make_float4(l2.L, l2.A, l2.B, 0.f);
    s_L[tid] = l2.L; s_A[tid] = l2.A; s_B[tid] = l2.B;
    s_gamma[tid] = g_tab.gamma[tid];
    s_gamma32[tid] = (float) g_tab.gamma[tid];
    __syncthreads();
    FastLookupLds r;
    r.S.argb = s_argb; r.S.lab = s_lab; r.S.gamma = s_gamma; r.S.gamma32 = s_gamma32; r.S.blue = g_tab.blue; r.S.path = nullptr;
    r.S.tileinfo = nullptr; r.S.stage = nullptr;
    r.pal.argb = s_argb; r.pal.L = s_L; r.pal.A = s_A; r.pal.B = s_B; r.pal.gamma = s_gamma; r.pal.blue = g_tab.blue;
    return r;
}
__device__ __forceinline__ FastLookup fast_lookup_ctx(const DevParams& P, const FastArgs& F) {
    FastLookup X;
    X.packed = F.packed; X.cont = F.cont; X.qa = F.qa; X.qb = F.qb; X.qc = F.qc;
    X.ratio = P.ratio; X.wr = P.PR * (1 - P.ratio); X.wg = P.PG * (1 - P.ratio); X.wb = P.PB * (1 - P.ratio);
    X.kfirst = P.hasAlpha ? 1 : 0;
    return X;
}
__device__ __forceinline__ int fast_nearest_any(const DevParams& P, const FastLookupLds& T, const FastLookup& X, const CellLists& lists, int c) {
    if (c_alpha(c) > 0xF) {
        const int cell = cell_of(c);
        const uint4 na = X.packed[2 * cell + 1];
        const int n = (int) (na.w >> 24);
        if (n != 255) return fast_nearest(T.S, X, c, na, n, cell);
    }
    return nearest_lab(P, T.pal, c, &lists);
}
__global__ void __launch_bounds__(256) fast_nearest_index_kernel(DevParams P, CellLists lists, FastArgs F, const int* __restrict__ g_palette,
                                                                 const int* __restrict__ colors, long long M, short* __restrict__ out) {
    const FastLookupLds T = fast_stage_lookup(P, g_palette);
    const FastLookup X = fast_lookup_ctx(P, F);
    for (long long i = (long long) blockIdx.x * blockDim.x + threadIdx.x; i < M; i += (long long) gridDim.x * blockDim.x)
        out[i] = (short) fast_nearest_any(P, T, X, lists, colors[i]);
}
__global__ void __launch_bounds__(256) fast_lookup_pass1_kernel(DevParams P, FastArgs F, const int* __restrict__ g_palette,
                                                                const int* __restrict__ pixels, long long N,
                                                                unsigned short* __restrict__ out_index, int* __restrict__ out_argb,
                                                                unsigned* __restrict__ todo ) {
    __shared__ __align__(16) int s_argb[256];
    __shared__ __align__(16) float4 s_lab[256];
    __shared__ float s_gamma32[256];
// ... 214 lines not shown
            const int* w = (const int*) A.in + 2 * i;
            const int c = A.which == NQ_FAST_ST_NEAR_D32 ? ((int) 0xFF000000 | (int) v) : w[0];
            const int k = (A.which == NQ_FAST_ST_NEAR_D32 ? (int) A.a0 : w[1]) & 255;
            float L, A1, B1;
            lab32_of(c, S.gamma32, L, A1, B1);
            A.out[i] = __float_as_uint(fast_near_d32(S.lab[k], L, A1, B1));
            break;
        }
        case NQ_FAST_ST_NEAR_SAFE: {
            const int* w = (const int*) A.in + 2 * i;
            uint4 na; na.x = (unsigned) w[1] & 0xFFFFu; na.y = na.z = na.w = 0u;
            bool safe;
            const int k1 = fast_nearest32(S, X, w[0], na, 2, 0, safe);
            A.out[i] = (unsigned) k1 | (safe ? 0x10000u : 0u);
            break;
        }
        default: break;
        }
    }
    if (counting && bad) {
        atomicAdd(reinterpret_cast<unsigned long long*>(A.out), bad);
        atomicMin(reinterpret_cast<unsigned long long*>(A.out) + 1, first_bad);
    }
}
}

namespace nq {

static const int8_t h_blue_fast[4096] = {
#include "../../include/nq_blue_noise_64x64.inc"
};
void upload_tables_fast(const double gamma[256], double exp1_5, double exp1_75, hipStream_t s) {
    ConstTables t;
    for (int i = 0; i < 256; ++i) t.gamma[i] = gamma[i];
    t.exp1_5 = exp1_5; t.exp1_75 = exp1_75;
    for (int i = 0; i < 4096; ++i) t.blue[i] = h_blue_fast[i];
    (void) hipMemcpyToSymbolAsync(HIP_SYMBOL(g_tab), &t, sizeof t, 0, hipMemcpyHostToDevice, s);
    (void) hipStreamSynchronize(s);
}

static inline CellLists to_lists_fast(const ListsView& v) {
    CellLists l; l.closest = v.closest; l.closestCount = v.closestCount; l.nearest = v.nearest; l.nearestCount = v.nearestCount;
    return l;
}

bool gilbert_fast_eligible(const DevParams& P, const GilbertConsts& G, const TileGeom& T, const ListsView& lv) {
    const int tilepx = T.tile_w * T.tile_h;
    const bool common = P.K > 32 && P.K <= 256 && !P.hasSemi && !P.rewriteA0 && !G.sortedByYDiff && !G.hasAlphaW && G.DITHER_MAX == 25 &&
                        fast_weights_match(G.weights) && lv.nearest && tilepx >= 1 && tilepx <= 1024 &&
                        fast_lds_bytes(tilepx, fast_stride_bytes(tilepx)) <= 160 * 1024 - 512;
    if (P.kind == 1) return common && lv.closest && P.ratio >= 0;
    return common && G.dither && !P.hasAlpha && !G.hasSaliencies;
}
bool fast_pack_wanted(const DevParams& P, const ListsView& lv) {
    return fast_lookup_eligible(P, lv) || (P.kind == 0 && P.K > 32 && P.K <= 256 && !P.hasSemi && !P.hasAlpha && lv.nearest && lv.closest);
}
void launch_pack_lists(const ListsView& lv, void* d_packed, hipStream_t s) {
    hipLaunchKernelGGL(pack_lists_kernel, dim3(65536 / 256), dim3(256), 0, s, to_lists_fast(lv), (uint4*) d_packed, (uint4*) d_packed + 2 * 65536);
}
static FastArgs fast_args(const DevParams& P, const ListsView& lv, void* d_packed, hipStream_t s) {
    FastArgs F;
    std::memset(&F, 0, sizeof F);
    double sq[3] = {0, 0, 0};
    static const float kc[3][3] = {{0.299f, 0.587f, 0.114f}, {-0.14713f, -0.28886f, 0.436f}, {0.615f, -0.51499f, -0.10001f}};
    for (int i = 0; i < 3; ++i) for (int c = 0; c < 3; ++c) sq[c] += (double) kc[i][c] * (double) kc[i][c];
    F.qa = (float) (P.PR * (1 - P.ratio) + P.ratio * sq[0]);
    F.qb = (float) (P.PG * (1 - P.ratio) + P.ratio * sq[1]);
    F.qc = (float) (P.PB * (1 - P.ratio) + P.ratio * sq[2]);
    F.packed = (const uint4*) d_packed;
    F.cont = F.packed + 2 * 65536;
    (void) lv; (void) s;
    return F;
}
hipError_t launch_gilbert_fast(const DevParams& P, const GilbertConsts& G, const TileGeom& T, const ListsView& lv, const int* d_pixels,
                               const float* d_saliency, const int* d_palette, long long seed, unsigned short* d_index, int* d_argb,
                               int* d_failed, void* d_packed, hipStream_t s, bool failed_cleared, bool chain_always) {
    const int ntiles = T.tiles_x * T.tiles_y;
    const int tilepx = T.tile_w * T.tile_h;
    FastArgs F = fast_args(P, lv, d_packed, s);
    F.limiterDiv = (float) (1 + std::sqrt((double) G.ditherMax));
    F.strideBytes = fast_stride_bytes(tilepx);
    F.failedCap = ntiles;
    F.failed = d_failed;
    F.chainAlways = chain_always ? 1 : 0;
#ifdef NQ_FAST_KNOCKOUT
    if (const char* e = std::getenv("NQ_FAST_DEBUG")) F.debug = std::atoi(e);
#endif
    F.vecOut = (T.tile_w % 4 == 0) && (T.width % 4 == 0) && ((uintptr_t) d_index % 8 == 0) && (!d_argb || (uintptr_t) d_argb % 16 == 0);
    hipError_t e = failed_cleared ? hipSuccess : hipMemsetAsync(d_failed, 0, sizeof(int), s);
    if (e != hipSuccess) return e;
    const size_t lds = fast_lds_bytes(tilepx, F.strideBytes);
    const int grid = (ntiles + 255) / 256;
    if (lds > 64 * 1024) {
        e = hipFuncSetAttribute((const void*) gilbert_fast_kernel<2, 1>, hipFuncAttributeMaxDynamicSharedMemorySize, 160 * 1024 - 512);
        if (e != hipSuccess) return e;
    }
    if (P.kind == 1)
        hipLaunchKernelGGL((gilbert_fast_kernel<2, 1>), dim3(grid), dim3(256), lds, s, P, G, T, to_lists_fast(lv), F, d_pixels, d_saliency, d_palette,
                           seed, d_index, d_argb);
    else {
        if (lds > 64 * 1024) {
            e = hipFuncSetAttribute((const void*) gilbert_fast_kernel<2, 0>, hipFuncAttributeMaxDynamicSharedMemorySize, 160 * 1024 - 512);
            if (e != hipSuccess) return e;
        }
        hipLaunchKernelGGL((gilbert_fast_kernel<2, 0>), dim3(grid), dim3(256), lds, s, P, G, T, to_lists_fast(lv), F, d_pixels, d_saliency, d_palette,
                           seed, d_index, d_argb);
    }
    return hipGetLastError();
}

bool fast_lookup_eligible(const DevParams& P, const ListsView& lv) {
    return P.kind == 1 && P.K > 32 && P.K <= 256 && !P.hasSemi && !P.rewriteA0 && lv.closest && lv.nearest && P.ratio >= 0;
}
static inline int fast_grid(int64_t n) { int64_t g = (n + 255) / 256; return (int) (g < 1 ? 1 : g > 256 * 16 ? 256 * 16 : g); }
void launch_fast_nearest_index(const DevParams& P, const ListsView& lv, const int* d_palette, void* d_packed, const int* d_colors, int64_t M,
                               short* d_out, hipStream_t s) {
    const FastArgs F = fast_args(P, lv, d_packed, s);
    hipLaunchKernelGGL(fast_nearest_index_kernel, dim3(fast_grid(M)), dim3(256), 0, s, P, to_lists_fast(lv), F, d_palette, d_colors, (long long) M, d_out);
}
void launch_fast_closest_tuple(const DevParams& P, const ListsView& lv, const int* d_palette, void* d_packed, const int* d_colors, int64_t M,
                               int* d_out4, hipStream_t s) {
    const FastArgs F = fast_args(P, lv, d_packed, s);
    hipLaunchKernelGGL(fast_closest_tuple_kernel, dim3(fast_grid(M)), dim3(256), 0, s, P, to_lists_fast(lv), F, d_palette, d_colors, (long long) M, d_out4);
}
void launch_fast_lookup_only(const DevParams& P, const ListsView& lv, const int* d_palette, void* d_packed, const int* d_pixels, int64_t N,
                             unsigned short* d_index, int* d_argb, unsigned* d_todo , hipStream_t s) {
    const FastArgs F = fast_args(P, lv, d_packed, s);
    (void) hipMemsetAsync(d_todo, 0, sizeof(unsigned), s);
    int64_t g1 = (N + 255) / 256;
    if (g1 > 256 * 32) g1 = 256 * 32;
    if (g1 < 1) g1 = 1;
    hipLaunchKernelGGL(fast_lookup_pass1_kernel, dim3((unsigned) g1), dim3(256), 0, s, P, F, d_palette, d_pixels, (long long) N, d_index, d_argb, d_todo);
    hipLaunchKernelGGL(fast_lookup_pass2_kernel, dim3(1024), dim3(256), 0, s, P, to_lists_fast(lv), F, d_palette, d_pixels, d_index, d_argb,
                       (const unsigned*) d_todo);
}
void launch_fast_bluenoise(const DevParams& P, const ListsView& lv, const int* d_palette, void* d_packed, const int* d_pixels, int width, int height,
                           int y_origin, float weight, long long seed, unsigned short* d_index, int* d_argb, hipStream_t s) {
    const FastArgs F = fast_args(P, lv, d_packed, s);
    hipLaunchKernelGGL(fast_bluenoise_kernel, dim3(fast_grid((int64_t) width * height)), dim3(256), 0, s, P, to_lists_fast(lv), F, d_palette, d_pixels,
                       width, height, y_origin, weight, seed, d_index, d_argb);
}

void launch_fast_selftest(const DevParams& P, const int* d_palette, int which, const void* d_in, int64_t first, int64_t n, int64_t a0, int64_t a1,
                          unsigned* d_out, hipStream_t s) {
    ListsView lv; std::memset(&lv, 0, sizeof lv);
// ... 19 lines not shown
```

### nquant.android_amd/csrc/nq_kernels.h

```cpp
#pragma once
#include <hip/hip_runtime.h>
#include <stdint.h>

namespace nq {

struct DevParams {
    int kind;
    int K;
    int hasSemi;
    int hasAlpha;
    int transparentColor;
    int isNano;
    int binKeyed;
    int nMaxColors;
    int rewriteA0;
    int pad;
    double PR, PG, PB, PA, ratio, weight;
};

struct GilbertConsts {
    int margin, thresold, DITHER_MAX, ditherMax, sortedByYDiff, hasAlphaW, dither;
    int hasSaliencies;
    int salSubst;
    float beta;
    double weightAbs;
    float weights[25];
    float w1[1], w3[3], w7[7], w15[15];
};

struct TileGeom {
    int width, height;
    int tile_w, tile_h, tiles_x, tiles_y;
    const uint32_t* path[4];
    int path_len[4];
    int shape_w[4], shape_h[4];
    int y_origin, tile_base;
};

void upload_tables(const double gamma[256], double exp1_5, double exp1_75, hipStream_t s);
void upload_tables_fast(const double gamma[256], double exp1_5, double exp1_75, hipStream_t s);

struct ListsView {
    const unsigned char* closest; const unsigned char* closestCount;
    const unsigned char* nearest; const unsigned char* nearestCount;
};
void launch_cell_lab_box(float* d_box , hipStream_t s);
struct SalJob { const int* pixels; long long N; float* out; long long vec4; int salSubst; int blocks; };
bool launch_build_lists(const DevParams& P, const int* d_palette, double wA, double wR, double wG, double wB, bool nearest,
                        const float* d_box, unsigned char* d_closest, unsigned char* d_closestCount, unsigned char* d_nearest,
                        unsigned char* d_nearestCount, hipStream_t s, const int* d_sal_pixels = nullptr, int64_t N = 0, float* d_sal_out = nullptr,
                        int salSubst = 0, void* d_packed = nullptr, int* d_failed = nullptr, bool* folded = nullptr);
void launch_saliency(const DevParams& P, int salSubst, const int* d_pixels, int64_t N, float* d_out, hipStream_t s);

void launch_nearest_index(const DevParams& P, const int* d_palette, const ListsView& lv, const int* d_colors, int64_t M, short* d_out, hipStream_t s);
void launch_closest_tuple(const DevParams& P, const int* d_palette, const ListsView& lv, const int* d_colors, int64_t M, int* d_out4, hipStream_t s);
void launch_lookup_only(const DevParams& P, const int* d_palette, const ListsView& lv, const int* d_pixels, int64_t N,
                        unsigned short* d_index, int* d_argb, hipStream_t s);

void launch_gilbert(const DevParams& P, const GilbertConsts& G, const TileGeom& T, const ListsView& lv, const int* d_pixels,
                    const float* d_saliency, const int* d_palette, short* d_binCache, long long seed, int sequential,
                    long long* d_rng_state, unsigned short* d_index, int* d_argb,
                    int* d_log, int* d_log_count, unsigned char* d_seen, int log_cap,
                    const int* d_tile_list, hipStream_t s);
bool gilbert_fast_eligible(const DevParams& P, const GilbertConsts& G, const TileGeom& T, const ListsView& lv);
hipError_t launch_gilbert_fast(const DevParams& P, const GilbertConsts& G, const TileGeom& T, const ListsView& lv, const int* d_pixels,
                               const float* d_saliency, const int* d_palette, long long seed, unsigned short* d_index, int* d_argb,
                               int* d_failed , void* d_packed , hipStream_t s,
                               bool failed_cleared = false ,
                               bool chain_always = false );
bool fast_lookup_eligible(const DevParams& P, const ListsView& lv);
bool fast_pack_wanted(const DevParams& P, const ListsView& lv);
void launch_pack_lists(const ListsView& lv, void* d_packed, hipStream_t s);
void launch_fast_nearest_index(const DevParams& P, const ListsView& lv, const int* d_palette, void* d_packed, const int* d_colors, int64_t M,
                               short* d_out, hipStream_t s);
void launch_fast_closest_tuple(const DevParams& P, const ListsView& lv, const int* d_palette, void* d_packed, const int* d_colors, int64_t M,
                               int* d_out4, hipStream_t s);
void launch_fast_lookup_only(const DevParams& P, const ListsView& lv, const int* d_palette, void* d_packed, const int* d_pixels, int64_t N,
                             unsigned short* d_index, int* d_argb, unsigned* d_todo, hipStream_t s);
void launch_fast_bluenoise(const DevParams& P, const ListsView& lv, const int* d_palette, void* d_packed, const int* d_pixels, int width, int height,
                           int y_origin, float weight, long long seed, unsigned short* d_index, int* d_argb, hipStream_t s);
void launch_fast_selftest(const DevParams& P, const int* d_palette, int which, const void* d_in, int64_t first, int64_t n, int64_t a0, int64_t a1,
                          unsigned* d_out, hipStream_t s);
void launch_bluenoise(const DevParams& P, const int* d_palette, const ListsView& lv, const int* d_pixels, int width, int height,
                      int y_origin ,
                      float weight, long long seed, int sequential, short* d_binCache, long long* d_rng_state,
                      unsigned short* d_index, int* d_argb, hipStream_t s);

struct Bins {
    float* f[4];
    double* d[4];
    float* cnt;
    float* err;
    int* nn;
    int* tm;
    int* mtm;
};
struct HistParams { int hasSemi, hasTransp, transparentColor, rewriteTransparent; };
struct NNParams {
    int kind, hasSemi, texicab;
    double ratio, PR, PG, PB, PA;
    int pgLessThanCoeff;
    double rgbTheta;
};
struct SortWorkspace {
    unsigned short *keys_a, *keys_b;
    int *vals_a, *vals_b;
    void* tmp; size_t tmp_bytes;
    unsigned *seg_start, *seg_end;
};
size_t sort_temp_bytes(int64_t n);
size_t sort32_temp_bytes(int64_t n, bool pairs);
void launch_distinct(const int* d_pixels, int64_t n, int transparentColor, unsigned* keys_a, unsigned* keys_b, unsigned* idx_a,
                     unsigned* idx_b, void* tmp, size_t tmp_bytes, unsigned long long* d_out, void* d_heads, unsigned cap, hipStream_t s);
void launch_color_presence(const int* d_pixels, int64_t n, int transparentColor, unsigned char* d_bytes, unsigned* d_set, unsigned slots,
                           unsigned* d_counters, hipStream_t s);
void launch_ciede_selftest(const float* d_pairs , int64_t n, unsigned* d_out , hipStream_t s);
void launch_prescan(const int* d_pixels, int64_t n, int64_t index_offset, long long* d_scan3, hipStream_t s);
bool launch_front(const int* d_pixels, int64_t n, long long* d_scan3, int* d_words , int defaultTransparent,
                  unsigned* d_occ_count, hipStream_t s);
struct FrameDesc { const int* pixels; long long n; long long offset; };
struct FrameChunk { int frame; int count; long long begin; };
#define NQ_FRAME_CHUNK 16384
// ... 152 lines not shown
```

### nquant.android_amd/host.py

```python
import ctypes as C
import os

import numpy as np

NQ_KIND_RGB, NQ_KIND_LAB = 0, 1
MODE_REFERENCE_SEQUENTIAL, MODE_PARALLEL_TILED, MODE_LOOKUP_ONLY = 0, 1, 2

_HERE = os.path.dirname(os.path.abspath(__file__))
_LIB = None

OPT_CELL_LISTS, OPT_FAST_DITHER, OPT_MERGE_WALL_SECONDS, OPT_DITHER_CHAIN = 1, 2, 3, 4
FAST_ST = {"TANH": (0, 2), "CLOSEST_ERR": (1, 3), "CLOSEST_ERR_PAIRS": (2, 3), "NEXTINT": (3, 1), "NEXTINT_COUNT": (4, 0), "REM": (5, 1),
           "REM_COUNT": (6, 0), "YDIFF": (7, 3), "YDIFF_RANGE": (8, 3), "LAB32": (9, 3), "LAB64": (10, 3), "NEAR_D32": (11, 1),
           "NEAR_D32_PAIRS": (12, 1), "TANH_BITS": (13, 2), "NEXTINT_LIST": (14, 1),
           "NEAR_SAFE": (15, 1)}
YDIFF_RECORD = np.dtype([("c1", np.int32), ("c2", np.int32), ("gt", np.int32), ("pad", np.int32), ("thr", np.float64)])


class NqError(RuntimeError):
    def __init__(self, status, message):
        super().__init__("nquant status %d: %s" % (status, message))
        self.status = status


class Params(C.Structure):
    _fields_ = [("kind", C.c_int32), ("nMaxColors", C.c_int32), ("hasSemiTransparency", C.c_int32),
                ("transparentPixelIndex", C.c_int32), ("transparentColor", C.c_int32), ("isNano", C.c_int32),
                ("texicab", C.c_int32), ("quan_rt", C.c_int32), ("maxbins", C.c_int32), ("paletteLength", C.c_int32),
                ("PR", C.c_double), ("PG", C.c_double), ("PB", C.c_double), ("PA", C.c_double),
                ("ratio", C.c_double), ("weight", C.c_double), ("distinctColors", C.c_int64)]

    def as_dict(self):
        return {f: getattr(self, f) for f, _ in self._fields_}


_vp, _i32, _i64 = C.c_void_p, C.c_int, C.c_int64
_pi32, _pi64, _pf32 = C.POINTER(C.c_int32), C.POINTER(C.c_int64), C.POINTER(C.c_float)
_ABI = {
    "nq_abi_version": (_i32, []),
    "nq_create": (_i32, [_i32, _i32, C.POINTER(_vp)]),
    "nq_destroy": (None, [_vp]),
    "nq_last_error": (C.c_char_p, [_vp]),
    "nq_set_stream": (_i32, [_vp, _vp]),
    "nq_set_tile": (_i32, [_vp, _i32, _i32]),
    "nq_set_option": (_i32, [_vp, _i32, _i32]),
    "nq_get_list_counts": (_i32, [_vp, _vp, _vp]),
    "nq_get_params": (_i32, [_vp, C.POINTER(Params)]),
    "nq_set_params": (_i32, [_vp, C.POINTER(Params)]),
    "nq_convert": (_i32, [_vp, _vp, _i32, _i32, _i32, _i32, _i64, _i32, _vp, _vp, _vp, _pi32]),
    "nq_convert_device": (_i32, [_vp, _vp, _i32, _i32, _i32, _i32, _i64, _i32, _vp, _vp, _vp, _pi32]),
    "nq_convert_batch_device": (_i32, [_vp, _i32, _vp, _vp, _vp, _i32, _i32, _vp, _i32, _vp, _vp, _vp, _i32, _vp]),
    "nq_convert_batch": (_i32, [_vp, _i32, _vp, _vp, _vp, _i32, _i32, _vp, _i32, _vp, _vp, _vp, _i32, _vp]),
    "nq_pnnquan": (_i32, [_vp, _vp, _i32, _i32, _i32, _vp, _pi32]),
    "nq_pnnquan_device": (_i32, [_vp, _vp, _i32, _i32, _i32, _vp, _pi32]),
    "nq_dither": (_i32, [_vp, _vp, _i32, _i32, _vp, _i32, _i32, _i64, _i32, _vp, _vp]),
    "nq_dither_device": (_i32, [_vp, _vp, _i32, _i32, _vp, _i32, _i32, _i64, _i32, _vp, _vp]),
    "nq_nearest_index": (_i32, [_vp, _vp, _i32, _vp, _i64, _vp]),
    "nq_closest_tuple": (_i32, [_vp, _vp, _i32, _vp, _i64, _vp]),
    "nq_band_scan_device": (_i32, [_vp, _vp, _i64, _i64, _i32, _vp]),
    "nq_set_scan": (_i32, [_vp, _i32, _i64, C.c_uint32, _i64]),
    "nq_band_histogram_device": (_i32, [_vp, _vp, _i64, _vp]),
    "nq_palette_from_histograms_device": (_i32, [_vp, _vp, _i32, _i32, _vp, _pi32]),
    "nq_band_distinct_device": (_i32, [_vp, _vp, _i64, _i32, _vp, _vp]),
    "nq_set_distinct": (_i32, [_vp, _i64, _vp]),
    "nq_get_stage_ms": (_i32, [_vp, _pf32]),
    "nq_get_merge_stats": (_i32, [_vp, _pi64]),
    "nq_get_batch_phase_ms": (_i32, [_vp, _pf32]),
    "nq_get_team_stats": (_i32, [_vp, _pi64]),
    "nq_get_merge_variant": (_i32, [_vp, _pi32, _pi32]),
    "nq_get_dither_path": (_i32, [_vp, _pi32, _pi32]),
    "nq_get_device_bytes": (_i32, [_pi64]),
    "nq_set_band": (_i32, [_vp, _i32, _i32]),
    "nq_selftest_ciede": (_i32, [_vp, _vp, _i64, _vp]),
    "nq_selftest_fast": (_i32, [_vp, _i32, _vp, _i64, _vp]),
    "nq_gilbert_dither": (_i32, [_vp, _i32, _i32, _vp, _vp, _i32, _vp, C.c_double, _i32, _i64, _i32, _vp, _vp]),
    "nq_bluenoise_dither": (_i32, [_vp, _i32, _i32, _vp, _vp, _i32, _vp, C.c_float, _i64, _i32, _vp]),
    "nq_band_color_presence_device": (_i32, [_vp, _vp, _i64, _vp, _i32, _pi64, _vp]),
    "nq_pnnquan_frames_device": (_i32, [_vp, _i32, _vp, _vp, _vp, _i32, _vp, _pi32]),
    "nq_convert_frames_device": (_i32, [_vp, _i32, _vp, _vp, _vp, _i32, _i32, _vp, _i32, _vp, _vp, _vp, _pi32]),
    "nq_convert_frames": (_i32, [_vp, _i32, _vp, _vp, _vp, _i32, _i32, _vp, _i32, _vp, _vp, _vp, _pi32]),
    "nq_gif_max_bytes": (_i32, [_i32, _vp, _vp, _i32, _i32, _pi64]),
    "nq_encode_gif_device": (_i32, [_vp, _i32, _vp, _vp, _vp, _vp, _i32, _vp, _i32, _i32, _vp, _i64, _pi64]),
    "nq_encode_gif": (_i32, [_vp, _i32, _vp, _vp, _vp, _vp, _i32, _vp, _i32, _i32, _vp, _i64, _pi64]),
    "nq_encode_gif_delta_device": (_i32, [_vp, _i32, _vp, _i32, _i32, _vp, _i32, _vp, _i32, _i32, _vp, _i64, _pi64, _vp]),
    "nq_encode_gif_delta": (_i32, [_vp, _i32, _vp, _i32, _i32, _vp, _i32, _vp, _i32, _i32, _vp, _i64, _pi64, _vp]),
    "nq_encode_gif_lossy_device": (_i32, [_vp, _i32, _vp, _vp, _vp, _vp, _i32, _vp, _i32, _i32, _i32, _vp, _i64, _pi64]),
    "nq_encode_gif_lossy": (_i32, [_vp, _i32, _vp, _vp, _vp, _vp, _i32, _vp, _i32, _i32, _i32, _vp, _i64, _pi64]),
    "nq_encode_gif_delta_lossy_device": (_i32, [_vp, _i32, _vp, _i32, _i32, _vp, _i32, _vp, _i32, _i32, _i32, _vp, _i64, _pi64, _vp]),
    "nq_encode_gif_delta_lossy": (_i32, [_vp, _i32, _vp, _i32, _i32, _vp, _i32, _vp, _i32, _i32, _i32, _vp, _i64, _pi64, _vp]),
    "nq_gif_local_max_bytes": (_i32, [_i32, _vp, _vp, _i32, _pi64]),
    "nq_encode_gif_local_device": (_i32, [_vp, _i32, _vp, _vp, _vp, _vp, _i32, _vp, _vp, _i32, _i32, _i32, _vp, _i64, _pi64]),
    "nq_encode_gif_local": (_i32, [_vp, _i32, _vp, _vp, _vp, _vp, _i32, _vp, _vp, _i32, _i32, _i32, _vp, _i64, _pi64]),
    "nq_encode_gif_local_delta_device": (_i32, [_vp, _i32, _vp, _i32, _i32, _vp, _i32, _vp, _vp, _i32, _i32, _i32, _vp, _i64, _pi64, _vp]),
    "nq_encode_gif_local_delta": (_i32, [_vp, _i32, _vp, _i32, _i32, _vp, _i32, _vp, _vp, _i32, _i32, _i32, _vp, _i64, _pi64, _vp]),
    "nq_png_max_bytes": (_i32, [_i32, _vp, _vp, _vp, _i32, _pi64]),
    "nq_encode_png_device": (_i32, [_vp, _i32, _vp, _vp, _vp, _vp, _i32, _vp, _i32, _vp, _i64, _vp]),
    "nq_encode_png": (_i32, [_vp, _i32, _vp, _vp, _vp, _vp, _i32, _vp, _i32, _vp, _i64, _vp]),
    "nq_apng_max_bytes": (_i32, [_i32, _i32, _i32, _i32, _pi64]),
    "nq_encode_apng_device": (_i32, [_vp, _i32, _vp, _i32, _i32, _vp, _i32, _vp, _i32, _i32, _vp, _i64, _pi64, _vp]),
    "nq_encode_apng": (_i32, [_vp, _i32, _vp, _i32, _i32, _vp, _i32, _vp, _i32, _i32, _vp, _i64, _pi64, _vp]),
    "nq_hold_frames_device": (_i32, [_vp, _i32, _vp, _vp, _vp, _i32, _i32, _i32, _vp]),
    "nq_hold_frames": (_i32, [_vp, _i32, _vp, _vp, _vp, _i32, _i32, _i32, _vp]),
    "nq_frame_signatures_device": (_i32, [_vp, _i32, _vp, _i32, _i32, _vp]),
    "nq_frame_signatures": (_i32, [_vp, _i32, _vp, _i32, _i32, _vp]),
    "nq_shots_from_signatures": (_i32, [_vp, _i32, _i64, _i32, _i32, _vp, _vp, _vp]),
    "nq_detect_shots_device": (_i32, [_vp, _i32, _vp, _i32, _i32, _i32, _i32, _vp, _vp, _vp]),
    "nq_detect_shots": (_i32, [_vp, _i32, _vp, _i32, _i32, _i32, _i32, _vp, _vp, _vp]),
    "nq_refine_palette_device": (_i32, [_vp, _i32, _vp, _vp, _vp, _vp, _i32, _i32, _vp, _vp, _pi32]),
    "nq_refine_palette": (_i32, [_vp, _i32, _vp, _vp, _vp, _vp, _i32, _i32, _vp, _vp, _pi32]),
    "nq_convert_frames_refined_device": (_i32, [_vp, _i32, _vp, _vp, _vp, _i32, _i32, _i32, _vp, _i32, _vp, _vp, _vp, _pi32]),
    "nq_convert_frames_refined": (_i32, [_vp, _i32, _vp, _vp, _vp, _i32, _i32, _i32, _vp, _i32, _vp, _vp, _vp, _pi32]),
    "nq_resample_frames_device": (_i32, [_vp, _i32, _vp, _i32, _i32, _i32, _i32, _i32, _i32, _vp, _i32, _i32, _i32]),
    "nq_resample_frames": (_i32, [_vp, _i32, _vp, _i32, _i32, _i32, _i32, _i32, _i32, _vp, _i32, _i32, _i32]),
    "nq_frames_from_yuv_device": (_i32, [_vp, _i32, _vp, _vp, _vp] + [_i32] * 6 + [_vp]),
    "nq_frames_from_yuv": (_i32, [_vp, _i32, _vp, _vp, _vp] + [_i32] * 6 + [_vp]),
    "nq_resample_frames_yuv_device": (_i32, [_vp, _i32, _vp, _vp, _vp] + [_i32] * 10 + [_vp, _i32, _i32, _i32]),
    "nq_resample_frames_yuv": (_i32, [_vp, _i32, _vp, _vp, _vp] + [_i32] * 10 + [_vp, _i32, _i32, _i32]),
    "nq_orient_frames_device": (_i32, [_vp, _i32, _vp, _i32, _i32, _i32, _vp]),
    "nq_orient_frames": (_i32, [_vp, _i32, _vp, _i32, _i32, _i32, _vp]),
    "nq_frames_from_yuv_oriented_device": (_i32, [_vp, _i32, _vp, _vp, _vp] + [_i32] * 7 + [_vp]),
    "nq_frames_from_yuv_oriented": (_i32, [_vp, _i32, _vp, _vp, _vp] + [_i32] * 7 + [_vp]),
    "nq_resample_frames_oriented_device": (_i32, [_vp, _i32, _vp] + [_i32] * 7 + [_vp, _i32, _i32, _i32]),
    "nq_resample_frames_oriented": (_i32, [_vp, _i32, _vp] + [_i32] * 7 + [_vp, _i32, _i32, _i32]),
    "nq_resample_frames_yuv_oriented_device": (_i32, [_vp, _i32, _vp, _vp, _vp] + [_i32] * 11 + [_vp, _i32, _i32, _i32]),
    "nq_resample_frames_yuv_oriented": (_i32, [_vp, _i32, _vp, _vp, _vp] + [_i32] * 11 + [_vp, _i32, _i32, _i32]),
    "nq_dither_ordered_device": (_i32, [_vp, _i32, _vp, _vp, _vp, _vp, _i32, _i32, _vp, _vp, _vp]),
    "nq_dither_ordered": (_i32, [_vp, _i32, _vp, _vp, _vp, _vp, _i32, _i32, _vp, _vp, _vp]),
    "nq_convert_frames_ordered_device": (_i32, [_vp, _i32, _vp, _vp, _vp, _i32, _i32, _i32, _vp, _vp, _vp, _pi32]),
    "nq_convert_frames_ordered": (_i32, [_vp, _i32, _vp, _vp, _vp, _i32, _i32, _i32, _vp, _vp, _vp, _pi32]),
    "nq_compare_frames_device": (_i32, [_i32, _vp, _i32, _vp, _vp, _vp, _vp, _i32, _vp]),
    "nq_compare_indexed_device": (_i32, [_i32, _vp, _i32, _vp, _vp, _vp, _i32, _vp, _vp, _i32, _vp]),
    "nq_compare_frames": (_i32, [_i32, _i32, _vp, _vp, _vp, _vp, _i32, _vp]),
    "nq_compare_indexed": (_i32, [_i32, _i32, _vp, _vp, _vp, _i32, _vp, _vp, _i32, _vp]),
    "nq_frames_from_yuv16_device": (_i32, [_i32, _vp, _i32, _vp, _vp, _vp] + [_i32] * 6 + [_vp]),
    "nq_frames_from_yuv16": (_i32, [_i32, _i32, _vp, _vp, _vp] + [_i32] * 6 + [_vp]),
    "nq_resample_frames_yuv16_device": (_i32, [_i32, _vp, _i32, _vp, _vp, _vp] + [_i32] * 10 + [_vp, _i32, _i32, _i32]),
    "nq_resample_frames_yuv16": (_i32, [_i32, _i32, _vp, _vp, _vp] + [_i32] * 10 + [_vp, _i32, _i32, _i32]),
    "nq_webp_max_bytes": (_i32, [_i32, _i32, _i32, _i32, _pi64]),
    "nq_encode_webp_device": (_i32, [_i32, _vp, _i32, _vp, _i32, _i32, _vp, _i32, _vp, _i32, _i32, _i32, _vp, _i64, _pi64, _vp]),
    "nq_encode_webp": (_i32, [_i32, _i32, _vp, _i32, _i32, _vp, _i32, _vp, _i32, _i32, _i32, _vp, _i64, _pi64, _vp]),
}


def abi_symbols():
    return list(_ABI)


def device_bytes():
    out = C.c_int64(0)
    rc = load_library().nq_get_device_bytes(C.byref(out))
    if rc != 0:
        raise NqError(rc, "nq_get_device_bytes")
    return out.value


def library_path():
    return os.environ.get("NQ_LIB") or os.path.join(_HERE, "libnquant_hip.so")


def _preload_hip_runtime():
    choice = os.environ.get("NQ_HIP_RUNTIME", "")
    if choice == "system":
        return
    cand = choice
    if not cand:
        try:
            import importlib.util
            spec = importlib.util.find_spec("torch")
            if spec is not None and spec.submodule_search_locations:
                cand = os.path.join(list(spec.submodule_search_locations)[0], "lib", "libamdhip64.so")
        except Exception:
            cand = ""
    if cand and os.path.exists(cand):
        C.CDLL(cand, mode=C.RTLD_GLOBAL)


def load_library():
    global _LIB
    if _LIB is not None:
        return _LIB
    path = library_path()
    if not os.path.exists(path):
        raise FileNotFoundError("%s is missing: run `python -c 'import __graft_entry__ as g; g.build()'`" % path)
    _preload_hip_runtime()
    L = C.CDLL(path)
    for name, (restype, argtypes) in _ABI.items():
        fn = getattr(L, name)
        fn.restype, fn.argtypes = restype, argtypes
    _LIB = L
    return L


def _as_i32(a):
    a = np.ascontiguousarray(a)
    if a.dtype == np.uint32:
        a = a.view(np.int32)
    if a.dtype != np.int32:
        raise TypeError("pixels must be int32/uint32 ARGB_8888, got %s" % a.dtype)
    return a


# ... 161 lines not shown
        self.ciede_quad_identical = (out[:, 8] >> 1) & 1
        return out[:, 0:4], out[:, 4:8], out[:, 8] & 1

    def selftest_fast(self, mode, first=None, count=None, a0=0, thresholds=None, gt=False, records=None):
        which, words = FAST_ST[mode]
        if records is None:
            thr = np.zeros(0) if thresholds is None else np.ascontiguousarray(thresholds, np.float64).reshape(-1)
            a1 = (thr.size << 1 | int(bool(gt))) if mode == "YDIFF_RANGE" else 0
            src = np.concatenate([np.array([first, count, a0, a1], np.int64), thr.view(np.int64)])
            n = int(count)
        else:
            src = np.ascontiguousarray(records, YDIFF_RECORD if mode == "YDIFF" else np.uint32 if mode == "TANH_BITS" else np.int32)
            n = src.shape[0]
        out = np.zeros((n, words) if words else 4, np.uint32)
        self._check(self._L.nq_selftest_fast(self._h, which, src.ctypes.data, n, out.ctypes.data))
        if words:
            return out
        bad, where = (int(v) for v in out.view(np.uint64))
        return bad, (None if where == 2 ** 64 - 1 else where)

    def nearestColorIndex(self, palette, colors):
        palette, colors = _as_i32(palette), _as_i32(colors).reshape(-1)
        out = np.empty(colors.size, np.int16)
        self._check(self._L.nq_nearest_index(self._h, palette.ctypes.data, len(palette), colors.ctypes.data, colors.size, out.ctypes.data))
        return out

    def closestTuple(self, palette, colors):
        palette, colors = _as_i32(palette), _as_i32(colors).reshape(-1)
        out = np.empty((colors.size, 4), np.int32)
        self._check(self._L.nq_closest_tuple(self._h, palette.ctypes.data, len(palette), colors.ctypes.data, colors.size, out.ctypes.data))
        return out

    def convert_device(self, d_pixels, nMaxColors, dither, d_out_argb, d_out_index=0, mode=None, seed=None):
        pal = np.zeros(max(int(nMaxColors), 2), np.int32)
        K = C.c_int32(0)
        self._check(self._L.nq_convert_device(self._h, C.c_void_p(d_pixels), self.width, self.height, int(nMaxColors), int(bool(dither)),
                                              int(self.seed if seed is None else seed), int(self.mode if mode is None else mode),
                                              C.c_void_p(d_out_argb), C.c_void_p(d_out_index or None), pal.ctypes.data, C.byref(K)))
        return pal[:K.value].copy()

    def pnnquan_device(self, d_pixels, nMaxColors):
        pal = np.zeros(max(int(nMaxColors), 2), np.int32)
        K = C.c_int32(0)
        self._check(self._L.nq_pnnquan_device(self._h, C.c_void_p(d_pixels), self.width, self.height, int(nMaxColors),
                                              pal.ctypes.data, C.byref(K)))
        return pal[:K.value].copy()

    def dither_device(self, d_pixels, palette, dither, d_out_argb, d_out_index=0, mode=None, seed=None):
        palette = _as_i32(palette)
        self._check(self._L.nq_dither_device(self._h, C.c_void_p(d_pixels), self.width, self.height, palette.ctypes.data, len(palette),
                                             int(bool(dither)), int(self.seed if seed is None else seed),
                                             int(self.mode if mode is None else mode), C.c_void_p(d_out_argb),
                                             C.c_void_p(d_out_index or None)))


def convert_batch_host(quantizers, pixels, nMaxColors, dither, out_argb, out_index=None, mode=None, seeds=None):
    return convert_batch_device(quantizers, pixels, nMaxColors, dither, out_argb, out_index, mode, seeds, _entry="nq_convert_batch")


def convert_batch_device(quantizers, d_pixels, nMaxColors, dither, d_out_argb, d_out_index=None, mode=None, seeds=None,
                         _entry="nq_convert_batch_device"):
    n = len(quantizers)
    if n == 0:
        return []
    q0 = quantizers[0]
    hs = (C.c_void_p * n)(*[q._h for q in quantizers])
    src = (C.c_void_p * n)(*[int(a) for a in d_pixels])
    dst = (C.c_void_p * n)(*[int(a) for a in d_out_argb])
    idx = (C.c_void_p * n)(*[int(a) for a in d_out_index]) if d_out_index is not None else None
    widths = np.array([q.width for q in quantizers], np.int32)
    heights = np.array([q.height for q in quantizers], np.int32)
    sd = np.array([q.seed for q in quantizers] if seeds is None else list(seeds), np.int64)
    stride = max(int(nMaxColors), 2)
    pal = np.zeros((n, stride), np.int32)
    K = np.zeros(n, np.int32)
    q0._check(getattr(q0._L, _entry)(hs, n, src, widths.ctypes.data, heights.ctypes.data, int(nMaxColors), int(bool(dither)),
                                            sd.ctypes.data, int(q0.mode if mode is None else mode), dst, idx, pal.ctypes.data,
                                            stride, K.ctypes.data))
    return [pal[i, :K[i]].copy() for i in range(n)]


def _frame_sizes(widths, heights, n):
    w = np.ascontiguousarray(widths, np.int32).reshape(-1)
    h = np.ascontiguousarray(heights, np.int32).reshape(-1)
    if w.size != n or h.size != n:
        raise ValueError("one width and one height per frame")
    return w, h


def pnnquan_frames_device(q, d_pixels, widths, heights, nMaxColors):
    n = len(d_pixels)
    w, h = _frame_sizes(widths, heights, n)
    src = (C.c_void_p * n)(*[int(a) for a in d_pixels])
    pal = np.zeros(max(int(nMaxColors), 2), np.int32)
    K = C.c_int32(0)
    q._check(q._L.nq_pnnquan_frames_device(q._h, n, src, w.ctypes.data, h.ctypes.data, int(nMaxColors), pal.ctypes.data, C.byref(K)))
    return pal[:K.value].copy()


def convert_frames_device(q, d_pixels, widths, heights, nMaxColors, dither, d_out_argb, d_out_index=None, mode=None, seeds=None):
    n = len(d_pixels)
    w, h = _frame_sizes(widths, heights, n)
    src = (C.c_void_p * n)(*[int(a) for a in d_pixels])
    dst = (C.c_void_p * n)(*[int(a) for a in d_out_argb])
    idx = (C.c_void_p * n)(*[int(a) or None for a in d_out_index]) if d_out_index is not None else None
    sd = np.array([q.seed] * n if seeds is None else list(seeds), np.int64)
# ... 71 lines not shown
```

Before: 8533.

## Split fast dither into light pass plus listed-tile chain on side stream

Adds a split mode for the fast Gilbert dither. A new light kernel handles tiles that need no saliency chain and records the tiles that do into a need list. A second fast-kernel pass then processes only those listed tiles, optionally on a side stream, so it can overlap with the next image in batched paths. The failed-tile buffer layout changes to hold the extra counter and list, and batch loops alternate scratch buffers and add event waits. This adds more launches and synchronisation complexity, and default activation depends on whether a chain stream is set (batch paths) and on the split eligibility conditions.

```diff
diff --git a/include/nquant_abi.h b/include/nquant_abi.h
--- a/include/nquant_abi.h
+++ b/include/nquant_abi.h
@@ -60,6 +60,7 @@
 #define NQ_OPT_MERGE_WALL_SECONDS 3
 int nq_set_option(nq_handle* h, int option, int value);
 int nq_get_dither_path(nq_handle* h, int32_t* out_fast, int32_t* out_failed_tiles);
+int nq_get_dither_split_stats(int64_t* out3);
 int nq_get_list_counts(nq_handle* h, uint8_t* closest_counts, uint8_t* nearest_counts);
 int nq_selftest_ciede(nq_handle* h, const float* lab_pairs, int64_t n, uint32_t* out9);
 #define NQ_FAST_ST_TANH 0
diff --git a/nquant.android_amd/csrc/nq_abi.cpp b/nquant.android_amd/csrc/nq_abi.cpp
--- a/nquant.android_amd/csrc/nq_abi.cpp
+++ b/nquant.android_amd/csrc/nq_abi.cpp
@@ -176,9 +176,13 @@
     DevBuf<float> d_user_sal;
     int band_y0 = 0, band_image_h = 0;
     int use_fast_dither = 1;
-    int dither_chain_always = 0;
+    int dither_chain = [] { const char* e = std::getenv("NQ_DITHER_CHAIN"); const int v = e ? std::atoi(e) : 0; return v >= 0 && v <= 3 ? v : 0; }();
+    hipStream_t chain_stream = nullptr;
+    hipEvent_t chain_gate = nullptr, chain_done = nullptr;
+    bool chain_on_side = false;
     bool dither_events_fresh = false;
     int last_dither_fast = 0;
+    bool split_uncounted = false;
     int last_dither_failed_tiles = 0;
     DevBuf<int> d_failed;
     DevBuf<float> scan_f;
@@ -274,6 +278,8 @@
         for (auto& e : ev) if (e) (void) hipEventDestroy(e);
         for (auto& e : bev) if (e) (void) hipEventDestroy(e);
         if (lane_gate) (void) hipEventDestroy(lane_gate);
+        if (chain_gate) (void) hipEventDestroy(chain_gate);
+        if (chain_done) (void) hipEventDestroy(chain_done);
         if (copy_stream) (void) hipStreamDestroy(copy_stream);
         if (lane_stream) (void) hipStreamDestroy(lane_stream);
         for (auto& ls : more_lanes) if (ls) (void) hipStreamDestroy(ls);
@@ -344,6 +350,9 @@
     h->palette_stream = h->stream; h->palette_synced = false;
     return NQ_OK;
 }
+static std::atomic<long long> g_split_passes{0}, g_split_side{0}, g_split_listed{0};
+int* failed_list(nq_handle* h) { return h->d_failed.p + 1; }
+size_t failed_words(const nq::TileGeom& T) { return 2 * ((size_t) T.tiles_x * T.tiles_y + 1); }
 void* packed_lists(nq_handle* h) { return h->sc->cell_lists.p + 2 * (size_t) 65536 * 32 + 2 * 65536; }
 
 int prepare_lists(nq_handle* h, const DevParams& P, nq::ListsView* out, const int* sal_pixels = nullptr, int64_t sal_n = 0, int sal_subst = 0,
@@ -957,8 +966,8 @@
     const bool want_sal = !staged && hasSal;
     const bool maybe_fast = !ov.blue_only && !sequential && h->use_fast_dither && K > 32 && K <= 256;
     bool failed_cleared = false;
-    if (maybe_fast) NQ_HIP(h, h->d_failed.reserve((size_t) T.tiles_x * T.tiles_y + 1));
-    { int rcl = lists_for_call(h, P, &lv, want_sal ? (const int*) d_argb : nullptr, n, salSubst ? 1 : 0, &sal_done, maybe_fast ? h->d_failed.p : nullptr,
+    if (maybe_fast) NQ_HIP(h, h->d_failed.reserve(failed_words(T)));
+    { int rcl = lists_for_call(h, P, &lv, want_sal ? (const int*) d_argb : nullptr, n, salSubst ? 1 : 0, &sal_done, maybe_fast ? failed_list(h) : nullptr,
                                &failed_cleared); if (rcl) return rcl; }
     const float* d_sal = nullptr;
     if (staged) d_sal = hasSal ? ov.d_sal : nullptr;
@@ -978,21 +987,34 @@
         NQ_HIP(h, hipMemsetAsync(h->d_seqseen.p, 0, (size_t) K, h->stream));
     }
     const int* d_tile_list = nullptr;
+    hipStream_t tail_stream = h->stream;
+    h->chain_on_side = false;
     h->last_dither_fast = 0;
+    h->split_uncounted = false;
     if (ov.blue_only) {  }
     else {
     if (!sequential && h->use_fast_dither && gilbert_fast_eligible(P, G, T, lv)) {
-        NQ_HIP(h, h->d_failed.reserve((size_t) T.tiles_x * T.tiles_y + 1));
+        NQ_HIP(h, h->d_failed.reserve(failed_words(T)));
+        int chain_mode = nq::FAST_CHAIN_FUSED;
+        if (h->dither_chain == 1) chain_mode = nq::FAST_CHAIN_ALWAYS;
+        else if (h->dither_chain == 3 || (h->dither_chain == 0 && h->chain_stream)) chain_mode = nq::FAST_CHAIN_SPLIT;
+        const bool split = chain_mode == nq::FAST_CHAIN_SPLIT && nq::gilbert_fast_split_eligible(P, G);
+        const bool side = split && h->chain_stream && h->chain_stream != h->stream;
+        if (split) ++g_split_passes;
+        if (side) ++g_split_side;
+        h->split_uncounted = split;
         NQ_HIP(h, launch_gilbert_fast(P, G, T, lv, (const int*) d_argb, d_sal, h->d_palette.p, (long long) seed, d_out_index,
-                                      post ? nullptr : (int*) d_out_argb, h->d_failed.p, packed_lists(h), h->stream, failed_cleared,
-                                      h->dither_chain_always != 0));
-        d_tile_list = h->d_failed.p;
+                                      post ? nullptr : (int*) d_out_argb, failed_list(h), packed_lists(h), h->stream, failed_cleared,
+                                      chain_mode, side ? h->chain_stream : nullptr, side ? h->chain_gate : nullptr));
+        if (side) tail_stream = h->chain_stream;
+        d_tile_list = failed_list(h);
         h->last_dither_fast = 1;
     }
     launch_gilbert(P, G, T, lv, (const int*) d_argb, d_sal, h->d_palette.p, h->d_bincache.p, (long long) seed, sequential ? 1 : 0,
                    h->d_scalars.p, d_out_index, post ? nullptr : (int*) d_out_argb,
                    seq_lab_post ? h->d_seqlog.p : nullptr, seq_lab_post ? h->d_seqlog.p + log_cap : nullptr,
-                   seq_lab_post ? h->d_seqseen.p : nullptr, log_cap, d_tile_list, h->stream);
+                   seq_lab_post ? h->d_seqseen.p : nullptr, log_cap, d_tile_list, tail_stream);
+    if (tail_stream != h->stream) { NQ_HIP(h, hipEventRecord(h->chain_done, tail_stream)); h->chain_on_side = true; }
     }
     rec(h, 6);
     if (seq_lab_post) {
@@ -1207,9 +1229,11 @@
     nq_handle* const* hs; int n;
     std::vector<hipStream_t> streams;
     std::vector<hipEvent_t> events;
+    hipStream_t side = nullptr;
     BatchGuard(nq_handle* const* hh, int nn) : hs(hh), n(nn) { for (int i = 0; i < n; ++i) streams.push_back(hs[i]->stream); }
     ~BatchGuard() {
-        for (int i = 0; i < n; ++i) { hs[i]->stream = streams[i]; hs[i]->sc = &hs[i]->own; hs[i]->light_events = false; }
+        if (side) (void) hipStreamSynchronize(side);
+        for (int i = 0; i < n; ++i) { hs[i]->stream = streams[i]; hs[i]->sc = &hs[i]->own; hs[i]->light_events = false; hs[i]->chain_stream = nullptr; }
         for (hipEvent_t e : events) (void) hipEventDestroy(e);
     }
 };
@@ -1311,7 +1335,7 @@
     if (!h) return NQ_ERR_INVALID;
     if (option == NQ_OPT_CELL_LISTS) { h->use_lists = value != 0; return NQ_OK; }
     if (option == NQ_OPT_FAST_DITHER) { h->use_fast_dither = value != 0; return NQ_OK; }
-    if (option == NQ_OPT_DITHER_CHAIN) { h->dither_chain_always = value != 0; return NQ_OK; }
+    if (option == NQ_OPT_DITHER_CHAIN) { h->dither_chain = value >= 0 && value <= 3 ? (int) value : 1; return NQ_OK; }
     if (option == NQ_OPT_MERGE_WALL_SECONDS) { h->merge_wall_s = value > 0 ? value : 0; return NQ_OK; }
     NQ_FAIL(h, NQ_ERR_INVALID, "unknown option %d", option);
 }
@@ -1382,11 +1406,17 @@
         *out_failed_tiles = 0;
         if (h->last_dither_fast && h->d_failed.p) {
             NQ_HIP(h, hipStreamSynchronize(h->stream));
-            int cnt = 0;
-            NQ_HIP(h, hipMemcpy(&cnt, h->d_failed.p, sizeof(int), hipMemcpyDeviceToHost));
-            *out_failed_tiles = cnt;
-        }
-    }
+            int cnt[2] = {0, 0};
+            NQ_HIP(h, hipMemcpy(cnt, h->d_failed.p, sizeof(cnt), hipMemcpyDeviceToHost));
+            *out_failed_tiles = cnt[1];
+            if (h->split_uncounted) { g_split_listed += cnt[0]; h->split_uncounted = false; }
+        }
+    }
+    return NQ_OK;
+}
+int nq_get_dither_split_stats(int64_t* out3) {
+    if (!out3) return NQ_ERR_INVALID;
+    out3[0] = g_split_passes.load(); out3[1] = g_split_side.load(); out3[2] = g_split_listed.load();
     return NQ_OK;
 }
 int nq_get_params(const nq_handle* h, nq_params* out) {
@@ -1633,6 +1663,24 @@
                       int nMaxColors, int dither, const int64_t* rng_seeds, int mode,
                       uint32_t* const* out_argb, uint16_t* const* out_index, uint32_t* out_palette, int32_t* out_K) {
     return nq_convert_frames_refined(h, n, argb, widths, heights, nMaxColors, 0, dither, rng_seeds, mode, out_argb, out_index, out_palette, out_K);
+}
+
+int finish_side_stream(nq_handle* h0, nq_handle* const* hs, int n, hipStream_t* side) {
+    *side = nullptr;
+    bool use_side = true;
+    if (const char* e = std::getenv("NQ_DITHER_SIDE_STREAM")) use_side = std::atoi(e) != 0;
+    if (!use_side) {
+        for (int i = 0; i < n; ++i) hs[i]->chain_stream = hs[i]->stream;
+        return NQ_OK;
+    }
+    if (!h0->lane_stream) NQ_HIP(h0, hipStreamCreateWithFlags(&h0->lane_stream, hipStreamNonBlocking));
+    for (int i = 0; i < n; ++i) {
+        if (!hs[i]->chain_gate) NQ_HIP(h0, hipEventCreateWithFlags(&hs[i]->chain_gate, hipEventDisableTiming));
+        if (!hs[i]->chain_done) NQ_HIP(h0, hipEventCreateWithFlags(&hs[i]->chain_done, hipEventDisableTiming));
+        hs[i]->chain_stream = h0->lane_stream;
+    }
+    *side = h0->lane_stream;
+    return NQ_OK;
 }
 
 int nq_convert_batch_device(nq_handle* const* hs, int n, const uint32_t* const* d_argb, const int32_t* widths, const int32_t* heights,
@@ -1739,12 +1787,22 @@
             rc = palette_check(hs[i], jobs[i], out_K + i);
             if (rc) return batch_fail(h0, hs[i], rc);
         }
+    hipStream_t side = nullptr;
+    rc = finish_side_stream(h0, hs, n, &side);
+    if (rc) return batch_fail(h0, h0, rc);
+    guard.side = side;
     for (int i = 0; i < n; ++i) {
         uint32_t* pal = out_palettes + (size_t) i * palette_stride;
+        if (side) {
+            hs[i]->sc = lane_sc[i & 1];
+            if (i >= 2 && hs[i - 2]->chain_on_side) NQ_HIP(h0, hipStreamWaitEvent(lane_s[0], hs[i - 2]->chain_done, 0));
+        }
         rc = dither_device(hs[i], d_argb[i], widths[i], heights[i], pal, out_K[i], dither, rng_seeds[i], mode, d_out_argb[i],
                            d_out_index ? d_out_index[i] : nullptr);
         if (rc) return batch_fail(h0, hs[i], rc);
     }
+    for (int i = std::max(0, n - 2); i < n; ++i)
+        if (hs[i]->chain_on_side) NQ_HIP(h0, hipStreamWaitEvent(lane_s[0], hs[i]->chain_done, 0));
     (void) hipEventRecord(h0->bev[3], lane_s[0]);
     NQ_HIP(h0, hipStreamSynchronize(lane_s[0]));
     for (int i = 0; i < n; ++i) finish_timing(hs[i]);
@@ -1806,6 +1864,10 @@
     if (rc) return rc;
     (void) hipEventRecord(h0->bev[2], h0->stream);
     for (int i = 0; i < n; ++i) if (jobs[i].merge) rec(hs[i], 4);
+    hipStream_t side = nullptr;
+    rc = finish_side_stream(h0, hs, n, &side);
+    if (rc) return batch_fail(h0, h0, rc);
+    guard.side = side;
     for (int i = 0; i < n; ++i) {
         uint32_t* pal = out_palettes + (size_t) i * palette_stride;
         if (jobs[i].merge) {
@@ -1814,17 +1876,24 @@
         }
         const int r = i % RING;
         if (i >= RING) NQ_HIP(h0, hipStreamWaitEvent(h0->stream, ev_dl[i - RING], 0));
+        if (side) {
+            hs[i]->sc = (i & 1) && n > 1 ? &hs[1]->own : &h0->own;
+            if (i >= 2 && hs[i - 2]->chain_on_side) NQ_HIP(h0, hipStreamWaitEvent(h0->stream, hs[i - 2]->chain_done, 0));
+        }
         rc = dither_device(hs[i], hs[i]->d_in.p, widths[i], heights[i], pal, out_K[i], dither, rng_seeds[i], mode,
                            (uint32_t*) h0->ring_argb[r].p, h0->ring_index[r].p);
         if (rc) return batch_fail(h0, hs[i], rc);
         NQ_HIP(h0, hipEventRecord(ev_done[i], h0->stream));
         NQ_HIP(h0, hipStreamWaitEvent(cs, ev_done[i], 0));
+        if (hs[i]->chain_on_side) NQ_HIP(h0, hipStreamWaitEvent(cs, hs[i]->chain_done, 0));
         const size_t px = (size_t) widths[i] * heights[i];
         NQ_HIP(h0, hipMemcpyAsync(out_argb[i], h0->ring_argb[r].p, px * sizeof(int), hipMemcpyDeviceToHost, cs));
         if (out_index && out_index[i])
             NQ_HIP(h0, hipMemcpyAsync(out_index[i], h0->ring_index[r].p, px * sizeof(uint16_t), hipMemcpyDeviceToHost, cs));
         NQ_HIP(h0, hipEventRecord(ev_dl[i], cs));
     }
+    for (int i = std::max(0, n - 2); i < n; ++i)
+        if (hs[i]->chain_on_side) NQ_HIP(h0, hipStreamWaitEvent(h0->stream, hs[i]->chain_done, 0));
     (void) hipEventRecord(h0->bev[3], h0->stream);
     NQ_HIP(h0, hipStreamSynchronize(h0->stream));
     NQ_HIP(h0, hipStreamSynchronize(cs));
diff --git a/nquant.android_amd/csrc/nq_dither.inc b/nquant.android_amd/csrc/nq_dither.inc
--- a/nquant.android_amd/csrc/nq_dither.inc
+++ b/nquant.android_amd/csrc/nq_dither.inc
@@ -156,7 +156,7 @@
                                                               unsigned char* __restrict__ nearest, unsigned char* __restrict__ nearestCount, SalJob sal,
                                                               void* packed, int* failed) {
     extern __shared__ __align__(16) unsigned char smem[];
-    if (failed && blockIdx.x == 0 && threadIdx.x == 0) failed[0] = 0;
+    if (failed && blockIdx.x == 0 && threadIdx.x == 0) { failed[-1] = 0; failed[0] = 0; }
     if (blockIdx.x < 256) closest_lists_body(P, g_palette, wA, wR, wG, wB, closest, closestCount, (int) blockIdx.x, packed);
     else if (blockIdx.x < 512) nearest_lists_body(P, g_palette, kstart, box, nearest, nearestCount, (int) blockIdx.x - 256, smem, packed);
     else saliency_body(P, sal.salSubst, sal.pixels, sal.N, sal.out, sal.vec4, (int) blockIdx.x - 512, sal.blocks, reinterpret_cast<double*>(smem));
diff --git a/nquant.android_amd/csrc/nq_dither_fast.hip b/nquant.android_amd/csrc/nq_dither_fast.hip
--- a/nquant.android_amd/csrc/nq_dither_fast.hip
+++ b/nquant.android_amd/csrc/nq_dither_fast.hip
@@ -1,6 +1,7 @@
 #include "nq_device.h"
 #include "nq_kernels.h"
 #include "../../include/nquant_abi.h"
+#include <algorithm>
 #include <cstring>
 #include <cmath>
 #include <cstdlib>
@@ -19,6 +20,9 @@
     const uint4* cont;
     int debug;
     int chainAlways;
+    int* needCount;
+    int* needTiles;
+    int listed;
 };
 #ifdef NQ_FAST_MARKS
 #define NQ_MARK(name) asm volatile("; MARK " name)
@@ -483,228 +487,8 @@
     return qidx;
 }
 
-template <int MINWAVES, int KIND = 1>
-__global__ void __launch_bounds__(256, MINWAVES) gilbert_fast_kernel(DevParams P, GilbertConsts G, TileGeom T, CellLists lists, FastArgs F,
-                                                                      const int* __restrict__ pixels, const float* __restrict__ saliency,
-                                                                      const int* __restrict__ g_palette, long long seed,
-                                                                      unsigned short* __restrict__ out_index, int* __restrict__ out_argb) {
-    extern __shared__ __align__(16) unsigned char smem[];
-    const int tilepx = T.tile_w * T.tile_h;
-    FastLds S;
-    {
-        unsigned char* p = smem;
-        S.argb = (const int*) p; p += 256 * 4;
-        S.lab = (const float4*) p; p += 256 * 16;
-        S.gamma = (const double*) p; p += 256 * 8;
-        S.gamma32 = (const float*) p; p += 256 * 4;
-        S.blue = (const signed char*) p; p += 4096;
-        S.path = (const unsigned*) p; p += (size_t) 4 * tilepx * 4;
-        S.tileinfo = (int4*) p; p += 256 * 16;
-        S.stage = p;
-    }
-    const int K = P.K;
-    const int tid = threadIdx.x;
-    {
-        int* a = (int*) S.argb; float4* l = (float4*) S.lab; double* g = (double*) S.gamma; float* g32 = (float*) S.gamma32;
-        int c2 = tid < K ? g_palette[tid] : 0;
-        a[tid] = c2;
-        if (KIND == 1) {
-            const Lab l2 = RGB2LAB(c2);
-            l[tid] = make_float4(l2.L, l2.A, l2.B, 0.f);
-        }
-        g[tid] = g_tab.gamma[tid];
-        g32[tid] = (float) g_tab.gamma[tid];
-        for (int i = tid; i < 1024; i += 256) ((int*) S.blue)[i] = ((const int*) g_tab.blue)[i];
-        unsigned* pp = (unsigned*) S.path;
-        for (int s = 0; s < 4; ++s)
-            for (int i = tid; i < tilepx; i += 256) pp[s * tilepx + i] = i < T.path_len[s] ? T.path[s][i] : 0u;
-    }
-
-    const int ntiles = T.tiles_x * T.tiles_y;
-    const int tile = blockIdx.x * 256 + tid;
-    const bool live = tile < ntiles;
-    const int ty = live ? tile / T.tiles_x : 0, tx = live ? tile - ty * T.tiles_x : 0;
-    const int shape = (tx == T.tiles_x - 1 ? 1 : 0) | (ty == T.tiles_y - 1 ? 2 : 0);
-    const int steps = live ? T.path_len[shape] : 0;
-    const int x0 = tx * T.tile_w, y0 = ty * T.tile_h;
-    S.tileinfo[tid] = make_int4(x0, y0, live ? T.shape_w[shape] : 0, live ? T.shape_h[shape] : 0);
-    __syncthreads();
-
-    const unsigned* __restrict__ path = S.path + shape * tilepx;
-    unsigned char* stage = S.stage + (size_t) tid * F.strideBytes;
-    const int width = T.width;
-    long long rng = jr_seed((long long) mix64((unsigned long long) seed + (unsigned long long) (T.tile_base + tile)));
-    const int gofs = T.y_origin * width;
-    const bool branchA = KIND == 1 && G.hasSaliencies && G.dither;
-    const bool hasSal = KIND == 1 && G.hasSaliencies != 0;
-    const double rpa = P.PA, rpr = P.PR, rpg = P.PG, rpb = P.PB;
-    FastLookup X;
-    X.packed = F.packed; X.cont = F.cont; X.qa = F.qa; X.qb = F.qb; X.qc = F.qc;
-    X.ratio = P.ratio; X.wr = P.PR * (1 - P.ratio); X.wg = P.PG * (1 - P.ratio); X.wb = P.PB * (1 - P.ratio);
-    X.kfirst = P.hasAlpha ? 1 : 0;
-    const float ditherMaxF = (float) G.ditherMax, ditherMax1 = (float) (G.ditherMax - 1);
-    const bool illusionAll = S.blue[0] > G.thresold;
-    bool failed = false;
-
-    unsigned d_next = 0;
-    int bidx_next = 0, pixel_next = 0;
-    float sal_next = 0.f;
-    const int maxsteps = T.path_len[0];
-
-    bool rewalk = true;
-    if (KIND == 1 && branchA && 2 * max(2, K - G.margin) > 100 && !F.chainAlways) {
-        rewalk = false;
-        if (steps > 0) {
-            d_next = path[0];
-            bidx_next = (x0 + (int) (d_next & 0xFFFFu)) + (y0 + (int) (d_next >> 16)) * width;
-            pixel_next = pixels[bidx_next];
-            sal_next = saliency[bidx_next];
-        }
-        for (int s = 0; s < maxsteps; ++s) {
-            bool need = false;
-            int c = 0, pos = 0;
-            if (s < steps) {
-                const int pixel = pixel_next;
-                const float sal = sal_next;
-                const int dxx = (int) (d_next & 0xFFFFu), dyy = (int) (d_next >> 16);
-                const int xx = x0 + dxx, yy = y0 + dyy + T.y_origin;
-                pos = dyy * T.tile_w + dxx;
-                if (s + 1 < steps) {
-                    d_next = path[s + 1];
-                    bidx_next = (x0 + (int) (d_next & 0xFFFFu)) + (y0 + (int) (d_next >> 16)) * width;
-                    pixel_next = pixels[bidx_next];
-                    sal_next = saliency[bidx_next];
-                }
-                NQ_MARK("light_begin");
-                need = K >= 256 && sal > .99f;
-                if (!need) c = fast_dither_color<true>(S, G, K, xx, yy, 0, pixel, sal, need);
-                NQ_MARK("light_color");
-            }
-            if (__ballot(need)) { rewalk = true; break; }
-            if (s < steps) {
-                const int qidx = fast_lab_index<true>(S, X, F, K, c, rng, failed);
-                stage[pos] = (unsigned char) qidx;
-                NQ_MARK("light_end");
-            }
-        }
-        NQ_COUNT(FC_CHAIN_LIGHT, live && !rewalk);
-        NQ_COUNT(FC_CHAIN_REWALK, live && rewalk);
-        if (rewalk) rng = jr_seed((long long) mix64((unsigned long long) seed + (unsigned long long) (T.tile_base + tile)));
-    }
-
-    float q[NQ_FQ][4];
-#pragma unroll
-    for (int t = 0; t < NQ_FQ; ++t) { q[t][0] = q[t][1] = q[t][2] = q[t][3] = 0.f; }
-
-    if (rewalk && steps > 0) {
-        d_next = path[0];
-        bidx_next = (x0 + (int) (d_next & 0xFFFFu)) + (y0 + (int) (d_next >> 16)) * width;
-        pixel_next = pixels[bidx_next];
-        if (hasSal) sal_next = saliency[bidx_next];
-    }
-    if (rewalk)
-    for (int s = 0; s < maxsteps; ++s) {
-        const int u = s % 5;
-        if (s < steps) {
-            const int bidx = bidx_next;
-            const int pixel = pixel_next;
-            const float sal = sal_next;
-            const int dxx = (int) (d_next & 0xFFFFu), dyy = (int) (d_next >> 16);
-            const int xx = x0 + dxx, yy = y0 + dyy + T.y_origin, pos = dyy * T.tile_w + dxx;
-            if (s + 1 < steps) {
-                d_next = path[s + 1];
-                bidx_next = (x0 + (int) (d_next & 0xFFFFu)) + (y0 + (int) (d_next >> 16)) * width;
-                pixel_next = pixels[bidx_next];
-                if (hasSal) sal_next = saliency[bidx_next];
-            }
-
-            NQ_MARK("step_begin");
-            float e[4] = {(float) c_red(pixel), (float) c_green(pixel), (float) c_blue(pixel), (float) c_alpha(pixel)};
-            float maxErr = 24.0f;
-            if (!NQ_KO(32))
-            switch (u) {
-                case 0: fast_accumulate<0>(q, e, maxErr); break;
-                case 1: fast_accumulate<1>(q, e, maxErr); break;
-                case 2: fast_accumulate<2>(q, e, maxErr); break;
-                case 3: fast_accumulate<3>(q, e, maxErr); break;
-                default: fast_accumulate<4>(q, e, maxErr); break;
-            }
-            const int r_pix = (int) fminf(255.0f, fmaxf(e[0], 0.0f));
-            const int g_pix = (int) fminf(255.0f, fmaxf(e[1], 0.0f));
-            const int b_pix = (int) fminf(255.0f, fmaxf(e[2], 0.0f));
-            const int a_pix = (int) fminf(255.0f, fmaxf(e[3], 0.0f));
-            const int c2 = c_argb(a_pix, r_pix, g_pix, b_pix);
-            NQ_MARK("accumulated");
-
-            int c = c2;
-            bool unused = false;
-            if (branchA && !(K >= 256 && sal > .99f) && !NQ_KO(8)) c = fast_dither_color<false>(S, G, K, xx, yy, c2, pixel, sal, unused);
-            NQ_MARK("dither_color");
-
-            int qidx = 0;
-            if (KIND == 0) {
-                if (c_alpha(c) != 255) failed = true;
-                else {
-                    const int cell = cell_of(c);
-                    const uint4 na = X.packed[2 * cell + 1];
-                    const int nnr = (int) (na.w >> 24);
-                    if (nnr == 255) failed = true;
-                    else qidx = fast_nearest_rgb(S, rpa, rpr, rpg, rpb, c, na, nnr, X.cont + 65536 + cell);
-                }
-            }
-            else qidx = fast_lab_index<false>(S, X, F, K, c, rng, failed);
-
-            const int cq = S.argb[qidx];
-            e[0] = (float) (r_pix - c_red(cq));
-            e[1] = (float) (g_pix - c_green(cq));
-            e[2] = (float) (b_pix - c_blue(cq));
-            e[3] = (float) (a_pix - c_alpha(cq));
-            const bool diffuse = S.blue[(bidx + gofs) & 4095] > G.thresold;
-            NQ_MARK("error_formed");
-            {
-                float ea = e[0], eb = e[1], ec = e[2];
-#pragma unroll 1
-                for (int j = 0; j < 3; ++j) {
-                    if (fabsf(ea) >= ditherMaxF && !NQ_KO(4)) {
-                        if (diffuse) ea = tanh_to_float(ea / maxErr * 20) * ditherMax1;
-                        else if (illusionAll) ea = (ea / maxErr) * ditherMax1;
-                        else ea /= F.limiterDiv;
-                    }
-                    const float tmp = ea; ea = eb; eb = ec; ec = tmp;
-                }
-                e[0] = ea; e[1] = eb; e[2] = ec;
-            }
-            NQ_MARK("limited");
-            switch (u) {
-                case 0: q[25][0] = e[0]; q[25][1] = e[1]; q[25][2] = e[2]; q[25][3] = e[3]; asm volatile("; push 0"); break;
-                case 1: q[26][0] = e[0]; q[26][1] = e[1]; q[26][2] = e[2]; q[26][3] = e[3]; asm volatile("; push 1"); break;
-                case 2: q[27][0] = e[0]; q[27][1] = e[1]; q[27][2] = e[2]; q[27][3] = e[3]; asm volatile("; push 2"); break;
-                case 3: q[28][0] = e[0]; q[28][1] = e[1]; q[28][2] = e[2]; q[28][3] = e[3]; asm volatile("; push 3"); break;
-                default:
-#pragma unroll
-                    for (int t = 0; t < 20; ++t) {
-#pragma unroll
-                        for (int j = 0; j < 4; ++j) q[t][j] = q[t + 5][j];
-                    }
-#pragma unroll
-                    for (int t = 20; t < 24; ++t) {
-#pragma unroll
-                        for (int j = 0; j < 4; ++j) q[t][j] = q[t + 5][j];
-                    }
-                    q[24][0] = e[0]; q[24][1] = e[1]; q[24][2] = e[2]; q[24][3] = e[3];
-                    break;
-            }
-            stage[pos] = (unsigned char) qidx;
-            NQ_MARK("step_end");
-        }
-    }
-
-    if (failed && live) {
-        const int slot = atomicAdd(F.failed, 1);
-        if (slot < F.failedCap) F.failed[1 + slot] = tile;
-    }
-    __syncthreads();
-
+__device__ __forceinline__ void fast_write_out(const FastLds& S, const FastArgs& F, const TileGeom& T, int tid, int width,
+                                               unsigned short* __restrict__ out_index, int* __restrict__ out_argb) {
     {
         const int wave = tid >> 6, lane = tid & 63;
         const unsigned char* wstage = S.stage + (size_t) (wave * 64) * F.strideBytes;
@@ -743,6 +527,342 @@
     }
 }
 
+template <int MINWAVES, int KIND = 1>
+__global__ void __launch_bounds__(256, MINWAVES) gilbert_fast_kernel(DevParams P, GilbertConsts G, TileGeom T, CellLists lists, FastArgs F,
+                                                                      const int* __restrict__ pixels, const float* __restrict__ saliency,
+                                                                      const int* __restrict__ g_palette, long long seed,
+                                                                      unsigned short* __restrict__ out_index, int* __restrict__ out_argb) {
+    extern __shared__ __align__(16) unsigned char smem[];
+    const int tilepx = T.tile_w * T.tile_h;
+    const int ntiles = T.tiles_x * T.tiles_y;
+    int nlisted = 0;
+    if (F.listed) {
+        nlisted = min(*F.needCount, min(F.failedCap, ntiles));
+        if ((int) blockIdx.x * 256 >= nlisted) return;
+    }
+    FastLds S;
+    {
+        unsigned char* p = smem;
+        S.argb = (const int*) p; p += 256 * 4;
+        S.lab = (const float4*) p; p += 256 * 16;
+        S.gamma = (const double*) p; p += 256 * 8;
+        S.gamma32 = (const float*) p; p += 256 * 4;
+        S.blue = (const signed char*) p; p += 4096;
+        S.path = (const unsigned*) p; p += (size_t) 4 * tilepx * 4;
+        S.tileinfo = (int4*) p; p += 256 * 16;
+        S.stage = p;
+    }
+    const int K = P.K;
+    const int tid = threadIdx.x;
+    {
+        int* a = (int*) S.argb; float4* l = (float4*) S.lab; double* g = (double*) S.gamma; float* g32 = (float*) S.gamma32;
+        int c2 = tid < K ? g_palette[tid] : 0;
+        a[tid] = c2;
+        if (KIND == 1) {
+            const Lab l2 = RGB2LAB(c2);
+            l[tid] = make_float4(l2.L, l2.A, l2.B, 0.f);
+        }
+        g[tid] = g_tab.gamma[tid];
+        g32[tid] = (float) g_tab.gamma[tid];
+        for (int i = tid; i < 1024; i += 256) ((int*) S.blue)[i] = ((const int*) g_tab.blue)[i];
+        unsigned* pp = (unsigned*) S.path;
+        for (int s = 0; s < 4; ++s)
+            for (int i = tid; i < tilepx; i += 256) pp[s * tilepx + i] = i < T.path_len[s] ? T.path[s][i] : 0u;
+    }
+
+    const int slot = blockIdx.x * 256 + tid;
+    int tile = slot;
+    bool live = slot < ntiles;
+    if (F.listed) {
+        live = slot < nlisted;
+        tile = live ? F.needTiles[slot] : 0;
+        live = live && tile >= 0 && tile < ntiles;
+    }
+    const int ty = live ? tile / T.tiles_x : 0, tx = live ? tile - ty * T.tiles_x : 0;
+    const int shape = (tx == T.tiles_x - 1 ? 1 : 0) | (ty == T.tiles_y - 1 ? 2 : 0);
+    const int steps = live ? T.path_len[shape] : 0;
+    const int x0 = tx * T.tile_w, y0 = ty * T.tile_h;
+    S.tileinfo[tid] = make_int4(x0, y0, live ? T.shape_w[shape] : 0, live ? T.shape_h[shape] : 0);
+    __syncthreads();
+
+    const unsigned* __restrict__ path = S.path + shape * tilepx;
+    unsigned char* stage = S.stage + (size_t) tid * F.strideBytes;
+    const int width = T.width;
+    long long rng = jr_seed((long long) mix64((unsigned long long) seed + (unsigned long long) (T.tile_base + tile)));
+    const int gofs = T.y_origin * width;
+    const bool branchA = KIND == 1 && G.hasSaliencies && G.dither;
+    const bool hasSal = KIND == 1 && G.hasSaliencies != 0;
+    const double rpa = P.PA, rpr = P.PR, rpg = P.PG, rpb = P.PB;
+    FastLookup X;
+    X.packed = F.packed; X.cont = F.cont; X.qa = F.qa; X.qb = F.qb; X.qc = F.qc;
+    X.ratio = P.ratio; X.wr = P.PR * (1 - P.ratio); X.wg = P.PG * (1 - P.ratio); X.wb = P.PB * (1 - P.ratio);
+    X.kfirst = P.hasAlpha ? 1 : 0;
+    const float ditherMaxF = (float) G.ditherMax, ditherMax1 = (float) (G.ditherMax - 1);
+    const bool illusionAll = S.blue[0] > G.thresold;
+    bool failed = false;
+
+    unsigned d_next = 0;
+    int bidx_next = 0, pixel_next = 0;
+    float sal_next = 0.f;
+    const int maxsteps = T.path_len[0];
+
+    bool rewalk = true;
+    if (KIND == 1 && branchA && 2 * max(2, K - G.margin) > 100 && !F.chainAlways) {
+        rewalk = false;
+        if (steps > 0) {
+            d_next = path[0];
+            bidx_next = (x0 + (int) (d_next & 0xFFFFu)) + (y0 + (int) (d_next >> 16)) * width;
+            pixel_next = pixels[bidx_next];
+            sal_next = saliency[bidx_next];
+        }
+        for (int s = 0; s < maxsteps; ++s) {
+            bool need = false;
+            int c = 0, pos = 0;
+            if (s < steps) {
+                const int pixel = pixel_next;
+                const float sal = sal_next;
+                const int dxx = (int) (d_next & 0xFFFFu), dyy = (int) (d_next >> 16);
+                const int xx = x0 + dxx, yy = y0 + dyy + T.y_origin;
+                pos = dyy * T.tile_w + dxx;
+                if (s + 1 < steps) {
+                    d_next = path[s + 1];
+                    bidx_next = (x0 + (int) (d_next & 0xFFFFu)) + (y0 + (int) (d_next >> 16)) * width;
+                    pixel_next = pixels[bidx_next];
+                    sal_next = saliency[bidx_next];
+                }
+                NQ_MARK("light_begin");
+                need = K >= 256 && sal > .99f;
+                if (!need) c = fast_dither_color<true>(S, G, K, xx, yy, 0, pixel, sal, need);
+                NQ_MARK("light_color");
+            }
+            if (__ballot(need)) { rewalk = true; break; }
+            if (s < steps) {
+                const int qidx = fast_lab_index<true>(S, X, F, K, c, rng, failed);
+                stage[pos] = (unsigned char) qidx;
+                NQ_MARK("light_end");
+            }
+        }
+        NQ_COUNT(FC_CHAIN_LIGHT, live && !rewalk);
+        NQ_COUNT(FC_CHAIN_REWALK, live && rewalk);
+        if (rewalk) rng = jr_seed((long long) mix64((unsigned long long) seed + (unsigned long long) (T.tile_base + tile)));
+    }
+
+    float q[NQ_FQ][4];
+#pragma unroll
+    for (int t = 0; t < NQ_FQ; ++t) { q[t][0] = q[t][1] = q[t][2] = q[t][3] = 0.f; }
+
+    if (rewalk && steps > 0) {
+        d_next = path[0];
+        bidx_next = (x0 + (int) (d_next & 0xFFFFu)) + (y0 + (int) (d_next >> 16)) * width;
+        pixel_next = pixels[bidx_next];
+        if (hasSal) sal_next = saliency[bidx_next];
+    }
+    if (rewalk)
+    for (int s = 0; s < maxsteps; ++s) {
+        const int u = s % 5;
+        if (s < steps) {
+            const int bidx = bidx_next;
+            const int pixel = pixel_next;
+            const float sal = sal_next;
+            const int dxx = (int) (d_next & 0xFFFFu), dyy = (int) (d_next >> 16);
+            const int xx = x0 + dxx, yy = y0 + dyy + T.y_origin, pos = dyy * T.tile_w + dxx;
+            if (s + 1 < steps) {
+                d_next = path[s + 1];
+                bidx_next = (x0 + (int) (d_next & 0xFFFFu)) + (y0 + (int) (d_next >> 16)) * width;
+                pixel_next = pixels[bidx_next];
+                if (hasSal) sal_next = saliency[bidx_next];
+            }
+
+            NQ_MARK("step_begin");
+            float e[4] = {(float) c_red(pixel), (float) c_green(pixel), (float) c_blue(pixel), (float) c_alpha(pixel)};
+            float maxErr = 24.0f;
+            if (!NQ_KO(32))
+            switch (u) {
+                case 0: fast_accumulate<0>(q, e, maxErr); break;
+                case 1: fast_accumulate<1>(q, e, maxErr); break;
+                case 2: fast_accumulate<2>(q, e, maxErr); break;
+                case 3: fast_accumulate<3>(q, e, maxErr); break;
+                default: fast_accumulate<4>(q, e, maxErr); break;
+            }
+            const int r_pix = (int) fminf(255.0f, fmaxf(e[0], 0.0f));
+            const int g_pix = (int) fminf(255.0f, fmaxf(e[1], 0.0f));
+            const int b_pix = (int) fminf(255.0f, fmaxf(e[2], 0.0f));
+            const int a_pix = (int) fminf(255.0f, fmaxf(e[3], 0.0f));
+            const int c2 = c_argb(a_pix, r_pix, g_pix, b_pix);
+            NQ_MARK("accumulated");
+
+            int c = c2;
+            bool unused = false;
+            if (branchA && !(K >= 256 && sal > .99f) && !NQ_KO(8)) c = fast_dither_color<false>(S, G, K, xx, yy, c2, pixel, sal, unused);
+            NQ_MARK("dither_color");
+
+            int qidx = 0;
+            if (KIND == 0) {
+                if (c_alpha(c) != 255) failed = true;
+                else {
+                    const int cell = cell_of(c);
+                    const uint4 na = X.packed[2 * cell + 1];
+                    const int nnr = (int) (na.w >> 24);
+                    if (nnr == 255) failed = true;
+                    else qidx = fast_nearest_rgb(S, rpa, rpr, rpg, rpb, c, na, nnr, X.cont + 65536 + cell);
+                }
+            }
+            else qidx = fast_lab_index<false>(S, X, F, K, c, rng, failed);
+
+            const int cq = S.argb[qidx];
+            e[0] = (float) (r_pix - c_red(cq));
+            e[1] = (float) (g_pix - c_green(cq));
+            e[2] = (float) (b_pix - c_blue(cq));
+            e[3] = (float) (a_pix - c_alpha(cq));
+            const bool diffuse = S.blue[(bidx + gofs) & 4095] > G.thresold;
+            NQ_MARK("error_formed");
+            {
+                float ea = e[0], eb = e[1], ec = e[2];
+#pragma unroll 1
+                for (int j = 0; j < 3; ++j) {
+                    if (fabsf(ea) >= ditherMaxF && !NQ_KO(4)) {
+                        if (diffuse) ea = tanh_to_float(ea / maxErr * 20) * ditherMax1;
+                        else if (illusionAll) ea = (ea / maxErr) * ditherMax1;
+                        else ea /= F.limiterDiv;
+                    }
+                    const float tmp = ea; ea = eb; eb = ec; ec = tmp;
+                }
+                e[0] = ea; e[1] = eb; e[2] = ec;
+            }
+            NQ_MARK("limited");
+            switch (u) {
+                case 0: q[25][0] = e[0]; q[25][1] = e[1]; q[25][2] = e[2]; q[25][3] = e[3]; asm volatile("; push 0"); break;
+                case 1: q[26][0] = e[0]; q[26][1] = e[1]; q[26][2] = e[2]; q[26][3] = e[3]; asm volatile("; push 1"); break;
+                case 2: q[27][0] = e[0]; q[27][1] = e[1]; q[27][2] = e[2]; q[27][3] = e[3]; asm volatile("; push 2"); break;
+                case 3: q[28][0] = e[0]; q[28][1] = e[1]; q[28][2] = e[2]; q[28][3] = e[3]; asm volatile("; push 3"); break;
+                default:
+#pragma unroll
+                    for (int t = 0; t < 20; ++t) {
+#pragma unroll
+                        for (int j = 0; j < 4; ++j) q[t][j] = q[t + 5][j];
+                    }
+#pragma unroll
+                    for (int t = 20; t < 24; ++t) {
+#pragma unroll
+                        for (int j = 0; j < 4; ++j) q[t][j] = q[t + 5][j];
+                    }
+                    q[24][0] = e[0]; q[24][1] = e[1]; q[24][2] = e[2]; q[24][3] = e[3];
+                    break;
+            }
+            stage[pos] = (unsigned char) qidx;
+            NQ_MARK("step_end");
+        }
+    }
+
+    if (failed && live) {
+        const int slot = atomicAdd(F.failed, 1);
+        if (slot < F.failedCap) F.failed[1 + slot] = tile;
+    }
+    __syncthreads();
+
+    fast_write_out(S, F, T, tid, width, out_index, out_argb);
+}
+
+__host__ __device__ __forceinline__ size_t light_lds_bytes(int tilepx, int strideBytes) { return fast_lds_bytes(tilepx, strideBytes) - 256 * 8; }
+__global__ void __launch_bounds__(256, 4) gilbert_light_kernel(DevParams P, GilbertConsts G, TileGeom T, FastArgs F,
+                                                               const int* __restrict__ pixels, const float* __restrict__ saliency,
+                                                               const int* __restrict__ g_palette, long long seed,
+                                                               unsigned short* __restrict__ out_index, int* __restrict__ out_argb) {
+    extern __shared__ __align__(16) unsigned char smem[];
+    const int tilepx = T.tile_w * T.tile_h;
+    FastLds S;
+    {
+        unsigned char* p = smem;
+        S.argb = (const int*) p; p += 256 * 4;
+        S.lab = (const float4*) p; p += 256 * 16;
+        S.gamma = g_tab.gamma;
+        S.gamma32 = (const float*) p; p += 256 * 4;
+        S.blue = (const signed char*) p; p += 4096;
+        S.path = (const unsigned*) p; p += (size_t) 4 * tilepx * 4;
+        S.tileinfo = (int4*) p; p += 256 * 16;
+        S.stage = p;
+    }
+    const int K = P.K;
+    const int tid = threadIdx.x;
+    {
+        int* a = (int*) S.argb; float4* l = (float4*) S.lab; float* g32 = (float*) S.gamma32;
+        const int c2 = tid < K ? g_palette[tid] : 0;
+        a[tid] = c2;
+        const Lab l2 = RGB2LAB(c2);
+        l[tid] = make_float4(l2.L, l2.A, l2.B, 0.f);
+        g32[tid] = (float) g_tab.gamma[tid];
+        for (int i = tid; i < 1024; i += 256) ((int*) S.blue)[i] = ((const int*) g_tab.blue)[i];
+        unsigned* pp = (unsigned*) S.path;
+        for (int s = 0; s < 4; ++s)
+            for (int i = tid; i < tilepx; i += 256) pp[s * tilepx + i] = i < T.path_len[s] ? T.path[s][i] : 0u;
+    }
+    const int ntiles = T.tiles_x * T.tiles_y;
+    const int tile = blockIdx.x * 256 + tid;
+    const bool live = tile < ntiles;
+    const int ty = live ? tile / T.tiles_x : 0, tx = live ? tile - ty * T.tiles_x : 0;
+    const int shape = (tx == T.tiles_x - 1 ? 1 : 0) | (ty == T.tiles_y - 1 ? 2 : 0);
+    const int steps = live ? T.path_len[shape] : 0;
+    const int x0 = tx * T.tile_w, y0 = ty * T.tile_h;
+    S.tileinfo[tid] = make_int4(x0, y0, live ? T.shape_w[shape] : 0, live ? T.shape_h[shape] : 0);
+    __syncthreads();
+
+    const unsigned* __restrict__ path = S.path + shape * tilepx;
+    unsigned char* stage = S.stage + (size_t) tid * F.strideBytes;
+    const int width = T.width;
+    long long rng = jr_seed((long long) mix64((unsigned long long) seed + (unsigned long long) (T.tile_base + tile)));
+    FastLookup X;
+    X.packed = F.packed; X.cont = F.cont; X.qa = F.qa; X.qb = F.qb; X.qc = F.qc;
+    X.ratio = P.ratio; X.wr = P.PR * (1 - P.ratio); X.wg = P.PG * (1 - P.ratio); X.wb = P.PB * (1 - P.ratio);
+    X.kfirst = P.hasAlpha ? 1 : 0;
+    bool failed = false, listed = false;
+    int left = steps;
+    unsigned d_next = 0;
+    int bidx_next = 0, pixel_next = 0;
+    float sal_next = 0.f;
+    const int maxsteps = T.path_len[0];
+    if (steps > 0) {
+        d_next = path[0];
+        bidx_next = (x0 + (int) (d_next & 0xFFFFu)) + (y0 + (int) (d_next >> 16)) * width;
+        pixel_next = pixels[bidx_next];
+        sal_next = saliency[bidx_next];
+    }
+    for (int s = 0; s < maxsteps; ++s) {
+        if (s < left) {
+            const int pixel = pixel_next;
+            const float sal = sal_next;
+            const int dxx = (int) (d_next & 0xFFFFu), dyy = (int) (d_next >> 16);
+            const int xx = x0 + dxx, yy = y0 + dyy + T.y_origin;
+            const int pos = dyy * T.tile_w + dxx;
+            if (s + 1 < steps) {
+                d_next = path[s + 1];
+                bidx_next = (x0 + (int) (d_next & 0xFFFFu)) + (y0 + (int) (d_next >> 16)) * width;
+                pixel_next = pixels[bidx_next];
+                sal_next = saliency[bidx_next];
+            }
+            bool need = K >= 256 && sal > .99f;
+            int c = 0;
+            if (!need) c = fast_dither_color<true>(S, G, K, xx, yy, 0, pixel, sal, need);
+            if (need) { listed = true; left = 0; }
+            else {
+                const int qidx = fast_lab_index<true>(S, X, F, K, c, rng, failed);
+                stage[pos] = (unsigned char) qidx;
+            }
+        }
+    }
+    NQ_COUNT_SUM(FC_CHAIN_LIGHT, live && !listed, 1);
+    NQ_COUNT_SUM(FC_CHAIN_REWALK, listed, 1);
+    if (listed) {
+        const int slot = atomicAdd(F.needCount, 1);
+        if (slot < F.failedCap) F.needTiles[slot] = tile;
+        S.tileinfo[tid] = make_int4(x0, y0, 0, 0);
+    }
+    else if (failed && live) {
+        const int slot = atomicAdd(F.failed, 1);
+        if (slot < F.failedCap) F.failed[1 + slot] = tile;
+    }
+    __syncthreads();
+    fast_write_out(S, F, T, tid, width, out_index, out_argb);
+}
 
 struct FastLookupLds { FastLds S; PalView pal; };
 __device__ __forceinline__ FastLookupLds fast_stage_lookup(const DevParams& P, const int* __restrict__ g_palette) {
@@ -1063,6 +1183,9 @@
     if (P.kind == 1) return common && lv.closest && P.ratio >= 0;
     return common && G.dither && !P.hasAlpha && !G.hasSaliencies;
 }
+bool gilbert_fast_split_eligible(const DevParams& P, const GilbertConsts& G) {
+    return P.kind == 1 && G.hasSaliencies && G.dither && 2 * std::max(2, P.K - G.margin) > 100;
+}
 bool fast_pack_wanted(const DevParams& P, const ListsView& lv) {
     return fast_lookup_eligible(P, lv) || (P.kind == 0 && P.K > 32 && P.K <= 256 && !P.hasSemi && !P.hasAlpha && lv.nearest && lv.closest);
 }
@@ -1085,7 +1208,8 @@
 }
 hipError_t launch_gilbert_fast(const DevParams& P, const GilbertConsts& G, const TileGeom& T, const ListsView& lv, const int* d_pixels,
                                const float* d_saliency, const int* d_palette, long long seed, unsigned short* d_index, int* d_argb,
-                               int* d_failed, void* d_packed, hipStream_t s, bool failed_cleared, bool chain_always) {
+                               int* d_failed, void* d_packed, hipStream_t s, bool failed_cleared, int chain_mode, hipStream_t chain_stream,
+                               hipEvent_t chain_gate) {
     const int ntiles = T.tiles_x * T.tiles_y;
     const int tilepx = T.tile_w * T.tile_h;
     FastArgs F = fast_args(P, lv, d_packed, s);
@@ -1093,15 +1217,45 @@
     F.strideBytes = fast_stride_bytes(tilepx);
     F.failedCap = ntiles;
     F.failed = d_failed;
-    F.chainAlways = chain_always ? 1 : 0;
+    F.chainAlways = chain_mode == FAST_CHAIN_ALWAYS ? 1 : 0;
+    F.needCount = d_failed - 1;
+    F.needTiles = d_failed + 1 + ntiles;
+    const bool split = chain_mode == FAST_CHAIN_SPLIT && gilbert_fast_split_eligible(P, G);
 #ifdef NQ_FAST_KNOCKOUT
     if (const char* e = std::getenv("NQ_FAST_DEBUG")) F.debug = std::atoi(e);
 #endif
     F.vecOut = (T.tile_w % 4 == 0) && (T.width % 4 == 0) && ((uintptr_t) d_index % 8 == 0) && (!d_argb || (uintptr_t) d_argb % 16 == 0);
-    hipError_t e = failed_cleared ? hipSuccess : hipMemsetAsync(d_failed, 0, sizeof(int), s);
+    hipError_t e = failed_cleared ? hipSuccess : hipMemsetAsync(d_failed - 1, 0, 2 * sizeof(int), s);
     if (e != hipSuccess) return e;
     const size_t lds = fast_lds_bytes(tilepx, F.strideBytes);
     const int grid = (ntiles + 255) / 256;
+    if (split) {
+        static const bool four = [] { const char* w = std::getenv("NQ_LIGHT_WAVES"); return w && std::atoi(w) == 4; }();
+        const size_t llds = light_lds_bytes(tilepx, F.strideBytes) + (four ? 256 * 8 : 0);
+        if (llds > 64 * 1024) {
+            e = hipFuncSetAttribute((const void*) gilbert_light_kernel, hipFuncAttributeMaxDynamicSharedMemorySize, 160 * 1024 - 512);
+            if (e != hipSuccess) return e;
+        }
+        hipLaunchKernelGGL(gilbert_light_kernel, dim3(grid), dim3(256), llds, s, P, G, T, F, d_pixels, d_saliency, d_palette, seed, d_index, d_argb);
+        e = hipGetLastError();
+        if (e != hipSuccess) return e;
+        hipStream_t cs = s;
+        if (chain_stream && chain_stream != s) {
+            e = hipEventRecord(chain_gate, s);
+            if (e == hipSuccess) e = hipStreamWaitEvent(chain_stream, chain_gate, 0);
+            if (e != hipSuccess) return e;
+            cs = chain_stream;
+        }
+        F.listed = 1;
+        F.chainAlways = 1;
+        if (lds > 64 * 1024) {
+            e = hipFuncSetAttribute((const void*) gilbert_fast_kernel<2, 1>, hipFuncAttributeMaxDynamicSharedMemorySize, 160 * 1024 - 512);
+            if (e != hipSuccess) return e;
+        }
+        hipLaunchKernelGGL((gilbert_fast_kernel<2, 1>), dim3(grid), dim3(256), lds, cs, P, G, T, to_lists_fast(lv), F, d_pixels, d_saliency, d_palette,
+                           seed, d_index, d_argb);
+        return hipGetLastError();
+    }
     if (lds > 64 * 1024) {
         e = hipFuncSetAttribute((const void*) gilbert_fast_kernel<2, 1>, hipFuncAttributeMaxDynamicSharedMemorySize, 160 * 1024 - 512);
         if (e != hipSuccess) return e;
diff --git a/nquant.android_amd/csrc/nq_kernels.h b/nquant.android_amd/csrc/nq_kernels.h
--- a/nquant.android_amd/csrc/nq_kernels.h
+++ b/nquant.android_amd/csrc/nq_kernels.h
@@ -63,11 +63,15 @@
                     int* d_log, int* d_log_count, unsigned char* d_seen, int log_cap,
                     const int* d_tile_list, hipStream_t s);
 bool gilbert_fast_eligible(const DevParams& P, const GilbertConsts& G, const TileGeom& T, const ListsView& lv);
+enum { FAST_CHAIN_FUSED = 0,
+       FAST_CHAIN_ALWAYS = 1,
+       FAST_CHAIN_SPLIT = 2 };
+bool gilbert_fast_split_eligible(const DevParams& P, const GilbertConsts& G);
 hipError_t launch_gilbert_fast(const DevParams& P, const GilbertConsts& G, const TileGeom& T, const ListsView& lv, const int* d_pixels,
                                const float* d_saliency, const int* d_palette, long long seed, unsigned short* d_index, int* d_argb,
-                               int* d_failed , void* d_packed , hipStream_t s,
+                               int* d_failed, void* d_packed , hipStream_t s,
                                bool failed_cleared = false ,
-                               bool chain_always = false );
+                               int chain_mode = FAST_CHAIN_FUSED, hipStream_t chain_stream = nullptr, hipEvent_t chain_gate = nullptr);
 bool fast_lookup_eligible(const DevParams& P, const ListsView& lv);
 bool fast_pack_wanted(const DevParams& P, const ListsView& lv);
 void launch_pack_lists(const ListsView& lv, void* d_packed, hipStream_t s);
diff --git a/nquant.android_amd/host.py b/nquant.android_amd/host.py
--- a/nquant.android_amd/host.py
+++ b/nquant.android_amd/host.py
@@ -1,4 +1,5 @@
 import ctypes as C
+import gc
 import os
 
 import numpy as np
@@ -69,6 +70,7 @@
     "nq_get_team_stats": (_i32, [_vp, _pi64]),
     "nq_get_merge_variant": (_i32, [_vp, _pi32, _pi32]),
     "nq_get_dither_path": (_i32, [_vp, _pi32, _pi32]),
+    "nq_get_dither_split_stats": (_i32, [_pi64]),
     "nq_get_device_bytes": (_i32, [_pi64]),
     "nq_set_band": (_i32, [_vp, _i32, _i32]),
     "nq_selftest_ciede": (_i32, [_vp, _vp, _i64, _vp]),
@@ -147,6 +149,7 @@
 
 
 def device_bytes():
+    gc.collect()
     out = C.c_int64(0)
     rc = load_library().nq_get_device_bytes(C.byref(out))
     if rc != 0:
@@ -414,6 +417,13 @@
                                              int(bool(dither)), int(self.seed if seed is None else seed),
                                              int(self.mode if mode is None else mode), C.c_void_p(d_out_argb),
                                              C.c_void_p(d_out_index or None)))
+
+
+def dither_split_stats():
+    out = (C.c_int64 * 3)()
+    if load_library().nq_get_dither_split_stats(out) != 0:
+        raise RuntimeError("nq_get_dither_split_stats failed")
+    return int(out[0]), int(out[1]), int(out[2])
 
 
 def convert_batch_host(quantizers, pixels, nMaxColors, dither, out_argb, out_index=None, mode=None, seeds=None):
```

Result: faster. 9616 (median of 6 runs) (+12.7%).
